# xissburg/edyn

Hardware: AMD Instinct MI355X
Metric: steps/sec (whole node), 32k-box pile, 10 SI iters; HBM GB/s in solve (higher is better)
Workload: dtype f32

## Files before the change

edyn_amd/_capi.py:

```python
import ctypes as C
import os
import numpy as np

_HERE = os.path.dirname(os.path.abspath(__file__))
LIB_PATH = os.environ.get("EDYNHIP_LIB") or os.path.join(_HERE, "libedynhip.so")


class EdynHipError(RuntimeError):
    def __init__(self, code, msg):
        super().__init__(f"edynhip error {code}: {msg}")
        self.code = code


class Config(C.Structure):
    _fields_ = [("device", C.c_int32), ("max_bodies", C.c_uint32), ("max_manifolds", C.c_uint32),
                ("max_joints", C.c_uint32), ("fixed_dt", C.c_float), ("num_velocity_iterations", C.c_uint32),
                ("num_position_iterations", C.c_uint32), ("gravity", C.c_float * 3), ("flags", C.c_uint32)]


class Bodies(C.Structure):
    _fields_ = [("kind", C.c_void_p), ("pos", C.c_void_p), ("orn", C.c_void_p), ("linvel", C.c_void_p),
                ("angvel", C.c_void_p), ("mass", C.c_void_p), ("inertia", C.c_void_p), ("has_inertia", C.c_void_p),
                ("shape_type", C.c_void_p), ("shape_param", C.c_void_p), ("friction", C.c_void_p),
                ("restitution", C.c_void_p), ("group", C.c_void_p), ("mask", C.c_void_p), ("gravity", C.c_void_p),
                ("sleeping_disabled", C.c_void_p), ("center_of_mass", C.c_void_p)]


class Joints(C.Structure):
    _fields_ = [("type", C.c_void_p), ("body", C.c_void_p), ("pivot", C.c_void_p), ("axis", C.c_void_p), ("params", C.c_void_p)]


class Params(C.Structure):
    _fields_ = [("fixed_dt", C.c_float), ("num_velocity_iterations", C.c_uint32), ("num_position_iterations", C.c_uint32),
                ("gravity", C.c_float * 3), ("num_restitution_iterations", C.c_uint32),
                ("num_individual_restitution_iterations", C.c_uint32)]


class Timings(C.Structure):
    _fields_ = [(n, C.c_float) for n in ("broadphase_ms", "narrowphase_ms", "islands_ms", "colouring_ms", "prepare_ms",
                                         "solve_velocity_ms", "integrate_ms", "solve_position_ms", "finish_ms", "step_ms")] + \
               [("solve_velocity_launches", C.c_uint32), ("steps", C.c_uint32)]


class Stats(C.Structure):
    _fields_ = [(n, C.c_uint32) for n in ("num_bodies", "num_manifolds", "num_points", "num_active_manifolds",
                                          "num_islands", "num_colours", "num_joint_colours", "colour_rounds",
                                          "num_joints", "num_joint_rows", "solve_schedule")] + [("colour_size", C.c_uint32 * 64)]


class WorldStats(C.Structure):
    _fields_ = [(n, C.c_uint32) for n in ("num_shards", "num_bodies", "steps", "approach_checks", "repartitions")] + [("bodies_per_shard", C.c_uint32 * 16), ("rebalances", C.c_uint32)]


class WorldEditStats(C.Structure):
    _fields_ = [(n, C.c_uint32) for n in ("edits", "in_place", "shard_rebuilds", "repartitions_by_edit", "approach_checks_by_edit")]


SCHEDULE_NAMES = {0: "none", 1: "k_contact_solve_df2 (dataflow, one launch per step, two lanes per manifold)",
                  2: "k_contact_solve_df (dataflow, one launch per step, one lane per manifold)",
                  3: "k_island_velocity (island-fused: one wave per island)",
                  4: "k_contact_solve_df2 + k_island_velocity (mixed: dataflow launch for islands without joints, one wave per jointed island)",
                  5: "k_contact_solve<WARM,PUSH> / k_joint_solve (one launch per colour and sweep)",
                  6: "k_contact_solve_df4 (dataflow, one launch per step, four lanes per manifold)"}


POINT_DTYPE = np.dtype([
    ("pivotA", np.float32, 3), ("pivotB", np.float32, 3), ("normal", np.float32, 3),
    ("local_normal", np.float32, 3), ("distance", np.float32), ("friction", np.float32),
    ("restitution", np.float32), ("attachment", np.int32), ("lifetime", np.uint32),
    ("normal_impulse", np.float32), ("friction_impulse", np.float32, 2)])
MANIFOLD_DTYPE = np.dtype([
    ("body", np.uint32, 2), ("num_points", np.uint32), ("colour", np.uint32), ("pt", POINT_DTYPE, 4)])

FLAG_TIMING, FLAG_SLEEPING, FLAG_EXCLUSIVE_DEVICE, FLAG_TIMING_SOLVE, FLAG_CONTACT_EVENTS = 1, 4, 8, 16, 32
FLAG_FUSED_VELOCITY_ROWS, FLAG_BLOCK_POSITION = 64, 128
PAIR_FILTER = C.CFUNCTYPE(C.c_int, C.c_void_p, C.c_uint32, C.c_uint32)
EVENT_DTYPE = np.dtype([("type", np.uint32), ("step", np.uint32), ("body", np.uint32, 2), ("point_id", np.uint64)])
EVENT_MANIFOLD_CREATED, EVENT_MANIFOLD_DESTROYED, EVENT_POINT_CREATED, EVENT_POINT_DESTROYED = 1, 2, 3, 4
RECORD_DTYPE = np.dtype([("pos", np.float32, 3), ("orn", np.float32, 4), ("linvel", np.float32, 3), ("angvel", np.float32, 3),
                         ("present_pos", np.float32, 3), ("present_orn", np.float32, 4), ("origin", np.float32, 3), ("flags", np.uint32)])
RECORD_DYNAMIC, RECORD_ASLEEP, RECORD_HAS_ORIGIN, RECORD_REMOVED = 1, 2, 4, 8
RAYCAST_HIT_DTYPE = np.dtype([("body", np.uint32), ("fraction", np.float32), ("normal", np.float32, 3), ("feature", np.int32),
                              ("feature_index", np.uint32), ("reserved", np.uint32)])
RAYCAST_NONE, RAYCAST_BOX_FACE, RAYCAST_CYLINDER_FACE, RAYCAST_CYLINDER_SIDE_EDGE = 0, 1, 2, 3
RAYCAST_CAPSULE_HEMISPHERE, RAYCAST_CAPSULE_SIDE, RAYCAST_POLYHEDRON_FACE = 4, 5, 6
RAYCAST_BRUTE_FORCE = 1
QUERY_PROCEDURAL, QUERY_NON_PROCEDURAL, QUERY_ISLANDS = 0, 1, 2
QUERY_CATEGORIES = {"procedural": QUERY_PROCEDURAL, "non_procedural": QUERY_NON_PROCEDURAL, "islands": QUERY_ISLANDS}
QUERY_BRUTE_FORCE = 1


class RecordView(C.Structure):
    _fields_ = [("records", C.c_void_p), ("num_bodies", C.c_uint32), ("step_index", C.c_uint32), ("events", C.c_void_p),
                ("num_events", C.c_uint32), ("total_events", C.c_uint32)]
STAGE_BROADPHASE, STAGE_NARROWPHASE, STAGE_ISLANDS, STAGE_SOLVE, STAGE_ALL = 1, 2, 4, 8, 15
PATH_BITS = {"COMPACT_DIRECT": 1 << 0, "COMPACT_LIBRARY": 1 << 1, "SORT_DIRECT": 1 << 2, "SORT_LIBRARY": 1 << 3, "SPECULATE": 1 << 4,
             "INPLACE": 1 << 5, "LISTS_FORCED": 1 << 6, "LOOKAHEAD_CHANGED": 1 << 7, "RELABEL_COMPRESS0": 1 << 8,
             "RELABEL_COMPRESS1": 1 << 9, "RELABEL_COMPRESSN": 1 << 10, "VEL_XCD": 1 << 11, "POS_XCD": 1 << 12, "VEL_LANES1": 1 << 13,
             "VEL_LANES2": 1 << 14, "VEL_LANES4": 1 << 15, "VEL_MULTI_ROUND": 1 << 16, "POS_MULTI_ROUND": 1 << 17,
             "POS_COLOUR_PUSH": 1 << 18, "MIXED": 1 << 19, "ISLAND_FUSED": 1 << 20, "PER_COLOUR": 1 << 21, "POLY_ONE_LANE": 1 << 22,
             "POLY_AXES8": 1 << 23, "POLY_AXES16": 1 << 24, "POLY_CONTACTS4": 1 << 25, "POLY_CONTACTS8": 1 << 26,
             "POLY_CONTACTS16": 1 << 27, "POLY_HINTS": 1 << 28, "RECORDS_DIRECT": 1 << 29, "RECORDS_COPY": 1 << 30,
             "WORLD_SERIAL": 1 << 31, "VEL_NAP": 1 << 32}

SYMBOLS = ["edynhip_create", "edynhip_destroy", "edynhip_last_error", "edynhip_set_stream", "edynhip_set_bodies",
           "edynhip_set_joints", "edynhip_step", "edynhip_run_stages", "edynhip_synchronize", "edynhip_get_state",
           "edynhip_set_state", "edynhip_pack_state_device", "edynhip_get_derived", "edynhip_num_manifolds",
           "edynhip_get_manifolds", "edynhip_set_manifolds", "edynhip_get_pairs", "edynhip_get_joint_impulses",
           "edynhip_get_timings", "edynhip_get_stats", "edynhip_abi_version", "edynhip_set_pair_filter", "edynhip_default_should_collide", "edynhip_debug_collide", "edynhip_add_bodies", "edynhip_get_asleep", "edynhip_wake_all", "edynhip_wake_bodies", "edynhip_set_center_of_mass",
           "edynhip_refresh_derived", "edynhip_exclude_collision", "edynhip_remove_collision_exclusion", "edynhip_add_joints",
           "edynhip_remove_joints", "edynhip_set_joint_params", "edynhip_remove_bodies", "edynhip_get_params", "edynhip_set_params",
           "edynhip_step_timed", "edynhip_get_contact_events", "edynhip_get_point_ids", "edynhip_snapshot", "edynhip_snapshot_read", "edynhip_snapshot_records", "edynhip_snapshot_map", "edynhip_set_event_prefetch", "edynhip_prefetched_events",
           "edynhip_set_material_extras", "edynhip_get_point_extras", "edynhip_set_joint_definition",
           "edynhip_set_generic_definition", "edynhip_get_joint_slot_impulses", "edynhip_set_material_ids", "edynhip_insert_material_mixing",
           "edynhip_measure_bandwidth", "edynhip_set_joint_warm_start", "edynhip_set_asleep", "edynhip_create_convex_mesh",
           "edynhip_get_convex_mesh",
           "edynhip_world_create", "edynhip_world_destroy", "edynhip_world_last_error", "edynhip_world_create_convex_mesh",
           "edynhip_world_set_bodies", "edynhip_world_set_joints", "edynhip_world_set_joint_definition", "edynhip_world_exclude_collision",
           "edynhip_world_step", "edynhip_world_get_state", "edynhip_world_get_partition", "edynhip_world_repartition",
           "edynhip_world_get_manifolds", "edynhip_world_get_stats", "edynhip_world_context", "edynhip_partition_islands",
           "edynhip_island_boxes_overlap", "edynhip_get_island_boxes",
           "edynhip_world_set_pair_filter", "edynhip_world_default_should_collide", "edynhip_get_sleep_timers", "edynhip_set_sleep_timers",
           "edynhip_raycast", "edynhip_raycast_device",
           "edynhip_query_aabb", "edynhip_query_aabb_device", "edynhip_query_aabb_stats",
           "edynhip_world_raycast", "edynhip_world_raycast_device", "edynhip_world_query_aabb", "edynhip_world_query_aabb_device",
           "edynhip_world_get_contact_events", "edynhip_world_get_point_ids",
           "edynhip_debug_paths", "edynhip_world_debug_paths",
           "edynhip_world_add_bodies", "edynhip_world_remove_bodies", "edynhip_world_add_joints", "edynhip_world_remove_joints",
           "edynhip_world_edit_joint", "edynhip_world_edit_exclusion", "edynhip_world_set_state", "edynhip_world_get_params",
           "edynhip_world_set_params", "edynhip_world_get_edit_stats", "edynhip_world_get_asleep"]

_lib = None


def lib():
    global _lib
    if _lib is None:
        if not os.path.exists(LIB_PATH):
            raise ImportError(f"{LIB_PATH} is missing - build it with __graft_entry__.build() (make -C edyn_amd/csrc); "
                              "there is no fallback path")
        L = C.CDLL(LIB_PATH)
        L.edynhip_create.restype = C.c_void_p
        L.edynhip_create.argtypes = [C.POINTER(Config), C.POINTER(C.c_int)]
        L.edynhip_destroy.argtypes = [C.c_void_p]
        L.edynhip_last_error.restype = C.c_char_p
        L.edynhip_last_error.argtypes = [C.c_void_p]
        L.edynhip_set_stream.argtypes = [C.c_void_p, C.c_void_p]
        L.edynhip_set_bodies.argtypes = [C.c_void_p, C.c_uint32, C.POINTER(Bodies)]
        L.edynhip_set_joints.argtypes = [C.c_void_p, C.c_uint32, C.POINTER(Joints)]
        L.edynhip_step.argtypes = [C.c_void_p, C.c_uint32]
        L.edynhip_run_stages.argtypes = [C.c_void_p, C.c_uint32]
        L.edynhip_synchronize.argtypes = [C.c_void_p]
        L.edynhip_get_state.argtypes = [C.c_void_p] + [C.c_void_p] * 4
        L.edynhip_set_state.argtypes = [C.c_void_p] + [C.c_void_p] * 4
        L.edynhip_pack_state_device.argtypes = [C.c_void_p, C.c_void_p, C.c_uint32, C.c_uint32]
        L.edynhip_get_derived.argtypes = [C.c_void_p] + [C.c_void_p] * 3
        L.edynhip_raycast.argtypes = [C.c_void_p, C.c_uint32, C.c_void_p, C.c_void_p, C.c_uint32, C.c_void_p, C.c_uint32, C.c_void_p]
        L.edynhip_raycast_device.argtypes = [C.c_void_p, C.c_uint32, C.c_void_p, C.c_void_p, C.c_uint32, C.c_void_p, C.c_uint32, C.c_void_p]
# ... 99 lines not shown
```

edyn_amd/csrc/capi.hip:

```cpp
#include "ctx.hpp"
#include "dpolyhedron.hpp"
#include <algorithm>
#include <atomic>
#include <chrono>
#include <cstdio>
#include <cstring>

namespace eh {
using namespace dm;

static std::string g_create_error;

int set_error(edynhip_ctx *c, int code, const char *what, hipError_t e) {
    std::string msg = what ? what : "";
    if (e != hipSuccess) { msg += ": "; msg += hipGetErrorString(e); }
    if (c) c->err = msg; else g_create_error = msg;
    return code;
}

namespace {
enum KnobKind { KNOB_ON, KNOB_OFF, KNOB_SET, KNOB_NUM, KNOB_PATH };
struct KnobRow {
    const char *name; KnobKind kind; long def;
    bool Knobs::*flag; long Knobs::*num; std::string Knobs::*path;
// ... 43 lines not shown
        case KNOB_SET: k.*r.flag = e != nullptr; break;
        case KNOB_NUM: k.*r.num = e ? atol(e) : r.def; break;
        case KNOB_PATH: k.*r.path = e ? e : ""; break;
        }
    }
    return k;
}

__global__ void k_publish_counters(const uint32_t *__restrict__ src, uint32_t *dst, uint32_t words, volatile uint32_t *seq, uint32_t value) {
    for (uint32_t i = threadIdx.x; i < words; i += blockDim.x) dst[i] = src[i];
    __threadfence_system();
    __syncthreads();
    if (threadIdx.x == 0) { __hip_atomic_store((uint32_t *)seq, value, __ATOMIC_RELEASE, __HIP_MEMORY_SCOPE_SYSTEM); }
}
int publish_counters(edynhip_ctx *c, size_t bytes, uint32_t *ticket) {
    const uint32_t value = ++c->cnt_seq_next;
    c->last_fetch_step = c->step_index;
    hipLaunchKernelGGL(k_publish_counters, dim3(1), dim3(256), 0, c->stream, (const uint32_t *)c->cnt, (uint32_t *)c->cnt_host,
                       (uint32_t)(bytes / sizeof(uint32_t)), c->cnt_seq, value);
    EH_HIP(c, hipGetLastError());
    *ticket = value;
    return EDYNHIP_OK;
}
int wait_counters(edynhip_ctx *c, uint32_t value) {
    const auto t0 = std::chrono::steady_clock::now();
    for (uint32_t spins = 0; *c->cnt_seq != value; ++spins) {
        __builtin_ia32_pause();
        if ((spins & 0xFFFFu) == 0xFFFFu && std::chrono::steady_clock::now() - t0 > std::chrono::seconds(2)) {
            EH_HIP(c, hipStreamSynchronize(c->stream));
            if (*c->cnt_seq != value) return set_error(c, EDYNHIP_ERR_INTERNAL, "fetch_counters: the published sequence number never arrived");
            break;
        }
    }
    std::atomic_thread_fence(std::memory_order_acquire);
    return EDYNHIP_OK;
}
int fetch_counters(edynhip_ctx *c, size_t bytes) {
    uint32_t ticket = 0;
    EH_TRY(publish_counters(c, bytes, &ticket));
    return wait_counters(c, ticket);
}

template <typename T>
static int dalloc(edynhip_ctx *c, T *&p, size_t count) {
    void *q = nullptr;
    size_t bytes = std::max<size_t>(count, 1) * sizeof(T);
    EH_HIP(c, hipMalloc(&q, bytes));
    EH_HIP(c, hipMemsetAsync(q, 0, bytes, c->stream));
    c->allocs.push_back(q);
    p = (T *)q;
    return EDYNHIP_OK;
}

static int alloc_manifolds(edynhip_ctx *c, Manifolds &m, uint32_t cap, uint32_t nb) {
    m.cap = cap;
    if (c->cfg.flags & EDYNHIP_FLAG_CONTACT_EVENTS) EH_TRY(dalloc(c, m.pid, (size_t)cap * kMaxPts));
    EH_TRY(dalloc(c, m.seg_start, nb)); EH_TRY(dalloc(c, m.seg_end, nb)); EH_TRY(dalloc(c, m.prev_idx, cap)); EH_TRY(dalloc(c, m.tree, cap));
    EH_TRY(dalloc(c, m.skey, cap)); EH_TRY(dalloc(c, m.bodyA, cap)); EH_TRY(dalloc(c, m.bodyB, cap)); EH_TRY(dalloc(c, m.info, cap));
    if (kPointRecords) {
        float4 *pts = nullptr;
        EH_TRY(dalloc(c, pts, (size_t)cap * kMaxPts * kPointF));
        m.pA = pts; m.pB = pts + 1; m.nrm = pts + 2; m.lnrm = pts + 3; m.imp = pts + 4;
    } else {
        EH_TRY(dalloc(c, m.pA, (size_t)cap * kMaxPts)); EH_TRY(dalloc(c, m.pB, (size_t)cap * kMaxPts));
        EH_TRY(dalloc(c, m.nrm, (size_t)cap * kMaxPts)); EH_TRY(dalloc(c, m.lnrm, (size_t)cap * kMaxPts));
        EH_TRY(dalloc(c, m.imp, (size_t)cap * kMaxPts));
    }
    return EDYNHIP_OK;
}

static int allocate(edynhip_ctx *c) {
    const uint32_t nb = c->cfg.max_bodies, M = c->cfg.max_manifolds, nj = c->cfg.max_joints;
    Bodies &b = c->b;
    b.cap = nb;
    EH_TRY(dalloc(c, b.xf, (size_t)nb * 8)); EH_TRY(dalloc(c, b.dvw, (size_t)nb * 2)); EH_TRY(dalloc(c, b.linvel, nb)); EH_TRY(dalloc(c, b.angvel, nb));
    EH_TRY(dalloc(c, b.amin, nb)); EH_TRY(dalloc(c, b.amax, nb)); EH_TRY(dalloc(c, b.shape, nb)); EH_TRY(dalloc(c, b.grav, nb));
    EH_TRY(dalloc(c, b.mat, nb)); EH_TRY(dalloc(c, b.mat2, nb)); EH_TRY(dalloc(c, b.flags, nb)); EH_TRY(dalloc(c, b.group, nb)); EH_TRY(dalloc(c, b.mask, nb));
    EH_TRY(dalloc(c, b.island, nb));
    EH_TRY(alloc_manifolds(c, c->m[0], M, nb));
    EH_TRY(alloc_manifolds(c, c->m[1], M, nb));
    Rows &r = c->rows;
    EH_TRY(dalloc(c, r.order, M)); EH_TRY(dalloc(c, r.bA, M)); EH_TRY(dalloc(c, r.bB, M)); EH_TRY(dalloc(c, r.np, M)); EH_TRY(dalloc(c, r.label, M));
    EH_TRY(dalloc(c, r.rw, (size_t)M * kMaxPts * kRowsPerPoint * kRowF));
    EH_TRY(dalloc(c, r.dslot, ((size_t)M + 64) * 4));
    EH_TRY(dalloc(c, r.pslot, ((size_t)M + 32) * 6));
    EH_TRY(dalloc(c, r.next, (size_t)M * 2)); EH_TRY(dalloc(c, r.im, (size_t)M * 2));
    EH_TRY(dalloc(c, r.pw, (size_t)M * kMaxPts * kPosF));
    EH_TRY(dalloc(c, r.slot_of, (size_t)nb * kMaxColours)); EH_TRY(dalloc(c, r.first_slot, nb)); EH_TRY(dalloc(c, r.skip, M));
    LBVH &t = c->bvh;
    EH_TRY(dalloc(c, t.keys, nb)); EH_TRY(dalloc(c, t.keys_sorted, nb));
    EH_TRY(dalloc(c, t.parent, (size_t)2 * nb)); EH_TRY(dalloc(c, t.left, nb)); EH_TRY(dalloc(c, t.right, nb));
    EH_TRY(dalloc(c, t.nmin, (size_t)2 * nb)); EH_TRY(dalloc(c, t.nmax, (size_t)2 * nb)); EH_TRY(dalloc(c, t.visit, nb));
    EH_TRY(dalloc(c, t.np_list, nb)); EH_TRY(dalloc(c, t.rope, (size_t)2 * nb)); EH_TRY(dalloc(c, t.split, 8));
    EH_TRY(dalloc(c, t.cand_list, (size_t)nb * kListCap)); EH_TRY(dalloc(c, t.cand_count, nb)); EH_TRY(dalloc(c, t.ref_min, nb)); EH_TRY(dalloc(c, t.ref_max, nb));
    EH_TRY(dalloc(c, c->np_ra, (size_t)M * kMaxPts)); EH_TRY(dalloc(c, c->np_rb, (size_t)M * kMaxPts)); EH_TRY(dalloc(c, c->np_rn, (size_t)M * kMaxPts));
    EH_TRY(dalloc(c, c->np_rnum, M));
    if (c->cfg.flags & EDYNHIP_FLAG_CONTACT_EVENTS) {
        c->event_cap = 5u * M + 1024u;
        EH_TRY(dalloc(c, c->events, c->event_cap)); EH_TRY(dalloc(c, c->event_count, 4)); EH_TRY(dalloc(c, c->prev_matched, M));
    }
    EH_TRY(dalloc(c, c->pair_keys, M)); EH_TRY(dalloc(c, c->pair_keys_sorted, M)); EH_TRY(dalloc(c, c->new_edges, M)); EH_TRY(dalloc(c, c->new_edge_m, M));
    EH_TRY(dalloc(c, c->isl_top, nb)); EH_TRY(dalloc(c, c->rot_off, nb)); EH_HIP(c, hipMemsetAsync(c->rot_off, 0xFF, (size_t)nb * sizeof(uint32_t), c->stream));
    EH_TRY(dalloc(c, c->own_keys, (size_t)nb * kOwnCap)); EH_TRY(dalloc(c, c->own_count, (size_t)nb + 1)); EH_TRY(dalloc(c, c->own_offset, (size_t)nb + 1));
    EH_TRY(dalloc(c, c->col_keys, M)); EH_TRY(dalloc(c, c->col_keys_sorted, M));
    EH_TRY(dalloc(c, c->col_unc, kColUncCap));
    { const size_t cs = 256 * (((size_t)M + 1023) / 1024) + 1; EH_TRY(dalloc(c, c->cs_hist, cs)); EH_TRY(dalloc(c, c->cs_start, cs)); EH_TRY(dalloc(c, c->cs_sup, 16 * 256)); EH_HIP(c, hipMemset(c->cs_sup, 0, 16 * 256 * sizeof(uint32_t))); }
    EH_TRY(dalloc(c, c->used, nb)); EH_TRY(dalloc(c, c->best[0], nb)); EH_TRY(dalloc(c, c->best[1], nb));
    EH_TRY(dalloc(c, c->com_store, nb)); EH_TRY(dalloc(c, c->origin_store, nb));
    EH_TRY(dalloc(c, c->isl_cnt, (size_t)nb + 1)); EH_TRY(dalloc(c, c->isl_off, (size_t)nb + 1)); EH_TRY(dalloc(c, c->isl_list, nb));
    EH_TRY(dalloc(c, c->isl_items, (size_t)M + nj)); EH_TRY(dalloc(c, c->isl_sorted, (size_t)M + nj)); EH_TRY(dalloc(c, c->isl_joint, nb));
    EH_TRY(dalloc(c, c->isl_err, nb)); EH_TRY(dalloc(c, c->isl_done, nb)); EH_TRY(dalloc(c, c->pos_err, (size_t)nb * kMaxDfPosIters));
    EH_TRY(dalloc(c, c->state_dev, (size_t)nb * 13));
    EH_HIP(c, hipHostMalloc((void **)&c->state_host, (size_t)nb * 13 * sizeof(float), hipHostMallocDefault));
    EH_TRY(dalloc(c, c->sleep_state, nb)); EH_TRY(dalloc(c, c->sleep_action, nb)); EH_TRY(dalloc(c, c->sleep_since, nb));
    EH_TRY(dalloc(c, c->sleep_old_label, nb)); EH_TRY(dalloc(c, c->sleep_size, nb)); EH_TRY(dalloc(c, c->sleep_best, nb)); EH_TRY(dalloc(c, c->sleep_carried, nb));
    EH_HIP(c, hipMemsetAsync(c->sleep_since, 0xFF, (size_t)nb * sizeof(double), c->stream));
    Joints &j = c->j;
    j.cap = nj;
    EH_TRY(dalloc(c, j.orig, nj)); EH_TRY(dalloc(c, j.type, nj)); EH_TRY(dalloc(c, j.bodyA, nj)); EH_TRY(dalloc(c, j.bodyB, nj));
    EH_TRY(dalloc(c, j.pivA, nj)); EH_TRY(dalloc(c, j.pivB, nj)); EH_TRY(dalloc(c, j.axA, nj)); EH_TRY(dalloc(c, j.pA, nj));
    EH_TRY(dalloc(c, j.qA, nj)); EH_TRY(dalloc(c, j.axB, nj)); EH_TRY(dalloc(c, j.pB, nj)); EH_TRY(dalloc(c, j.impulse, (size_t)nj * kJointSlots));
    EH_TRY(dalloc(c, j.wbx, nj)); EH_TRY(dalloc(c, j.gJ, (size_t)nj * 18)); EH_TRY(dalloc(c, j.params, (size_t)nj * kJointParams)); EH_TRY(dalloc(c, j.angle, nj)); EH_TRY(dalloc(c, j.rmask, nj));
    EH_TRY(dalloc(c, j.rA, nj)); EH_TRY(dalloc(c, j.rB, nj)); EH_TRY(dalloc(c, j.wp, nj)); EH_TRY(dalloc(c, j.wq, nj)); EH_TRY(dalloc(c, j.wax, nj));
    EH_TRY(dalloc(c, j.eff, (size_t)nj * kJointSlots)); EH_TRY(dalloc(c, j.rhs, (size_t)nj * kJointSlots));
    EH_TRY(dalloc(c, j.lo, (size_t)nj * kJointSlots)); EH_TRY(dalloc(c, j.hi, (size_t)nj * kJointSlots));
    c->sort_tmp_bytes = sort_temp_bytes(std::max(std::max(M, nb + 1), 256u * ((M + 1023u) / 1024u) + 1u));
    { void *q = nullptr; EH_HIP(c, hipMalloc(&q, c->sort_tmp_bytes)); c->allocs.push_back(q); c->sort_tmp = q; }
    EH_TRY(dalloc(c, c->cnt, 1));
    EH_HIP(c, hipHostMalloc((void **)&c->cnt_host, sizeof(Counters), hipHostMallocDefault));
    std::memset(c->cnt_host, 0, sizeof(Counters));
    { void *q = nullptr; EH_HIP(c, hipHostMalloc(&q, 64, hipHostMallocDefault)); std::memset(q, 0, 64); c->cnt_seq = (volatile uint32_t *)q; }
    EH_HIP(c, hipStreamSynchronize(c->stream));
    return EDYNHIP_OK;
}

struct RawBodies {
    const int32_t *kind; const float *pos, *orn, *linvel, *angvel, *mass, *inertia; const uint8_t *has_inertia;
    const int32_t *shape_type; const float *shape_param, *friction, *restitution; const uint64_t *group, *mask; const float *gravity; const uint8_t *sleeping_disabled; const float *com;
};
__global__ void k_init_bodies(uint32_t first, uint32_t n, RawBodies r, Bodies b, float3 default_gravity, dc::Meshes meshes) {
    const uint32_t l = blockIdx.x * blockDim.x + threadIdx.x;
    if (l >= n) return;
    const uint32_t i = first + l;
    const int kind = r.kind[l], st = r.shape_type[l];
    const f3 pos = mk3(r.pos[3 * l], r.pos[3 * l + 1], r.pos[3 * l + 2]);
    const q4 orn{r.orn[4 * l], r.orn[4 * l + 1], r.orn[4 * l + 2], r.orn[4 * l + 3]};
    const float4 sp = make_float4(r.shape_param[4 * l], r.shape_param[4 * l + 1], r.shape_param[4 * l + 2], r.shape_param[4 * l + 3]);
    float inv_m = 0;
    m3 il = m3_zero(), iw = m3_zero();
    const f3 com = r.com ? mk3(r.com[3 * l], r.com[3 * l + 1], r.com[3 * l + 2]) : mk3(0, 0, 0);
    const bool has_com = !(com.x == 0 && com.y == 0 && com.z == 0);
    if (kind == EDYNHIP_KIND_DYNAMIC) {
        const float mass = r.mass[l];
        inv_m = 1.0f / mass;
        m3 I;
        if (r.has_inertia && r.has_inertia[l]) {
            const float *p = r.inertia + 9 * l;
            I = {{p[0], p[1], p[2]}, {p[3], p[4], p[5]}, {p[6], p[7], p[8]}};
        } else if (st == dc::SHAPE_BOX) {
            f3 ext = from4(sp) * 2.0f;
            f3 d = 1.0f / 12.0f * mass * mk3(ext.y * ext.y + ext.z * ext.z, ext.z * ext.z + ext.x * ext.x, ext.x * ext.x + ext.y * ext.y);
            I = {{d.x, 0, 0}, {0, d.y, 0}, {0, 0, d.z}};
        } else if (st == dc::SHAPE_SPHERE) {
            float s = 0.4f * mass * sp.x * sp.x;
            I = {{1 * s, 0 * s, 0 * s}, {0 * s, 1 * s, 0 * s}, {0 * s, 0 * s, 1 * s}};
        } else if (st == dc::SHAPE_CAPSULE) {
// ... 1689 lines not shown
```

edyn_amd/csrc/ctx.hpp:

```cpp
#pragma once
#include <hip/hip_runtime.h>
#include <cstdint>
#include <functional>
#include <string>
#include <array>
#include <map>
#include <vector>
#include "../../include/edynhip.h"
#include "dmesh.hpp"

namespace eh {

constexpr uint32_t kNoColour = 0xFFu;
constexpr uint32_t kMaxColours = 64;
constexpr uint32_t kMaxContactColours = 63;
constexpr uint32_t kSerialColour = 62;
constexpr int kMaxPts = 4;

constexpr uint32_t BF_KIND_MASK = 0x3u;
constexpr uint32_t BF_SHAPE_SHIFT = 4;
constexpr uint32_t BF_SHAPE_MASK = 0xF0u;
constexpr uint32_t BF_ASLEEP = 0x100u;
constexpr uint32_t BF_NOSLEEP = 0x200u;
constexpr uint32_t BF_REMOVED = 0x400u;
// ... 29 lines not shown
    uint32_t *seg_start = nullptr, *seg_end = nullptr;
    uint32_t *prev_idx = nullptr;
    uint8_t *tree = nullptr;
    float4 *pA = nullptr;
    float4 *pB = nullptr;
    float4 *nrm = nullptr;
    float4 *lnrm = nullptr;
    float4 *imp = nullptr;
    uint64_t *pid = nullptr;
    float4 *xmat = nullptr;
    float4 *ximp = nullptr;
};
constexpr bool kPointRecords = true;
constexpr int kPointF = 5;
__host__ __device__ __forceinline__ size_t pt_at(uint32_t cap, uint32_t k, uint32_t m) {
    return kPointRecords ? ((size_t)m * 4 + k) * kPointF : (size_t)k * cap + m;
}
__host__ __device__ __forceinline__ size_t slot_at(uint32_t cap, uint32_t k, uint32_t m) { return (size_t)k * cap + m; }
constexpr int kXRowF = 3, kXRows = 3, kXPoint = kXRows * kXRowF + 1;

__device__ __forceinline__ const float *mix_lookup(const Bodies &b, uint32_t body0, uint32_t body1) {
    if (b.mix_K == 0) return nullptr;
    const uint32_t c0 = b.mat_cid[body0], c1 = b.mat_cid[body1];
    if (c0 == 0xFFFFFFFFu || c1 == 0xFFFFFFFFu) return nullptr;
    const int32_t e = b.mix_lut[(size_t)c0 * b.mix_K + c1];
    return e < 0 ? nullptr : b.mix_vals + 6 * (size_t)e;
}

struct ContactEvent { uint32_t type, step, bodyA, bodyB; uint64_t pid; };
struct EventSink { ContactEvent *buf; uint32_t *count; uint32_t cap; uint32_t step; uint32_t tag; };
__device__ __forceinline__ void emit_event(const EventSink &ev, uint32_t type, uint32_t a, uint32_t b, uint64_t pid) {
    const uint32_t i = atomicAdd(ev.count, 1u);
    if (i < ev.cap) ev.buf[i] = ContactEvent{type, ev.step, a, b, pid};
}

constexpr int kJointSlots = 24, kJointParams = 64, kJointApiParams = 10, kJointApiSlots = 9, kJointBaseSlots = 9;
struct Joints {
    uint32_t n = 0, cap = 0, num_colours = 0, rows = 0;
    uint32_t *orig = nullptr;
    uint32_t *type = nullptr, *bodyA = nullptr, *bodyB = nullptr;
    float4 *pivA = nullptr, *pivB = nullptr;
    float4 *axA = nullptr;
    float4 *pA = nullptr, *qA = nullptr;
    float4 *axB = nullptr, *pB = nullptr;
    float *params = nullptr;
    float *angle = nullptr;
    float *impulse = nullptr;
    float4 *rA = nullptr, *rB = nullptr;
    float4 *wp = nullptr, *wq = nullptr;
    float4 *wax = nullptr;
    float4 *wbx = nullptr;
    float4 *gJ = nullptr;
    float *eff = nullptr, *rhs = nullptr;
    float *lo = nullptr, *hi = nullptr;
    uint32_t *rmask = nullptr;
    uint32_t colour_start[kMaxColours + 1] = {0};
};
struct HostJoint {
    int32_t type = 0;
    uint32_t body[2] = {0, 0};
    float pivot[6] = {0}, axis[6] = {0};
    float frame[18] = {0};
    bool has_frames = false;
    float params[kJointParams] = {0};
    float impulse[kJointSlots] = {0};
    float angle = 0;
    bool alive = true;
};

struct Rows {
    uint32_t *order = nullptr;
    uint32_t *bA = nullptr, *bB = nullptr, *np = nullptr;
    uint32_t *label = nullptr;
    float4 *rw = nullptr;
    float4 *rwx = nullptr;
    float4 *dslot = nullptr;
    uint32_t *next = nullptr;
    float4 *pslot = nullptr;
    float *im = nullptr;
    float4 *pw = nullptr;
    uint32_t *slot_of = nullptr;
    uint32_t *first_slot = nullptr;
    uint8_t *skip = nullptr;
};
constexpr int kRowF = 5, kRowsPerPoint = 3, kPosF = 4;
constexpr uint32_t kColUncCap = 16384;
constexpr uint32_t kHeadBit = 0x80000000u, kSlotMask = 0x7FFFFFFFu;
__host__ __device__ inline size_t dslot_at(uint32_t slot, uint32_t half) {
    const uint32_t p = slot >> 1, side = slot & 1u;
    return ((size_t)(p >> 6) << 8) + (((side << 1) + half) << 6) + (p & 63u);
}
__host__ __device__ inline size_t pslot_at(uint32_t slot, uint32_t piece) {
    const uint32_t p = slot >> 1;
    return (size_t)(p >> 5) * 192u + (piece << 6) + (slot & 63u);
}

struct Knobs {
    bool dataflow, dataflow_pos, island_fused, mixed, df_xcd;
    long df_lanes, df_waves, dfp_waves, df_nap;
    std::string df_trace, dfp_trace;
    long df_trace_step;
    bool speculate, inplace, bp_lists, bp_adapt, direct_compact, direct_sort, col_lds, np_fused;
    long cc_compress;
    bool poly_hint;
    long poly_group, poly_group2;
    long query_scan_ratio, records_direct;
    bool world_serial, world_trace;
    bool bp_stats, pp_prof, tree_stats;
};

struct RayTree;
struct QueryAabb;

struct LBVH {
    uint64_t *keys = nullptr, *keys_sorted = nullptr;
    uint32_t *parent = nullptr;
    uint32_t *left = nullptr, *right = nullptr;
    uint32_t *rope = nullptr;
    uint32_t *split = nullptr;
    uint32_t *cand_list = nullptr, *cand_count = nullptr;
    float4 *ref_min = nullptr, *ref_max = nullptr;
    bool lists_dirty = true;
    float lookahead = 6.0f;
    uint32_t rebuild_hist = 0;
    float4 *nmin = nullptr, *nmax = nullptr;
    uint32_t *visit = nullptr;
    uint32_t *np_list = nullptr;
    uint32_t num_proc = 0, num_np = 0;
    uint32_t age = 0;
};

struct CandLists { uint32_t *list; uint32_t *count; float4 *ref_min, *ref_max; };
constexpr uint32_t kListCap = 128;
constexpr int kOwnCap = 64;
constexpr uint32_t kListOverflow = 0xFFFFFFFFu;

constexpr uint32_t kMaxDfPosIters = 8;

struct Counters {
    uint32_t num_pairs;
    uint32_t pair_overflow;
    uint32_t num_points;
    uint32_t num_active;
    uint32_t uncoloured;
    uint32_t colour_overflow;
    uint32_t num_islands;
    uint32_t pairs_changed;
    uint32_t num_found;
    uint32_t num_new;
    uint32_t num_extra;
    uint32_t num_awake;
    uint32_t unc_count;
    uint32_t bp_rebuild;
    uint32_t df_abort;
    uint32_t pairs_differ;
    uint32_t isl_num;
    uint32_t isl_max_items;
    uint32_t isl_max_jitems;
    uint32_t isl_free;
    uint32_t tree_found;
    uint32_t tree_marks;
    uint32_t tree_total;
    uint32_t col_wg_rounds;
    uint32_t bp_rebuilt;
    int32_t bounds_min[3], bounds_max[3];
    uint32_t colour_start[4 * kMaxColours], colour_end[4 * kMaxColours];
// ... 213 lines not shown
```

edyn_amd/csrc/solver.hip:

```cpp
#include <mutex>
#include "dstep.hpp"
#include "dpolyhedron.hpp"

namespace eh {

struct BRef { f3 pos, org; q4 orn; f3 v, w; float inv_m; m3 inv_I; };
DI BRef load_bref(const Bodies &b, uint32_t i) {
    BRef r;
    float4 p = B_POS(b, i);
    uint32_t fl = b.flags[i];
    r.pos = from4(p); r.org = B_ORG(b, i); r.orn = q_from4(B_ORN(b, i));
    if (is_dynamic(fl)) {
        r.inv_m = p.w;
        r.inv_I = {from4(B_IW(b, i, 0)), from4(B_IW(b, i, 1)), from4(B_IW(b, i, 2))};
    } else { r.inv_m = 0; r.inv_I = m3_zero(); }
    if ((fl & BF_KIND_MASK) == EDYNHIP_KIND_STATIC) { r.v = mk3(0, 0, 0); r.w = mk3(0, 0, 0); }
    else { r.v = from4(b.linvel[i]); r.w = from4(b.angvel[i]); }
    return r;
}
DI float eff_mass(f3 J0, f3 J1, f3 J2, f3 J3, float imA, const m3 &iA, float imB, const m3 &iB) {
    float s = dot(J0, J0) * imA + dot(mul(iA, J1), J1) + dot(J2, J2) * imB + dot(mul(iB, J3), J3);
    return 1.0f / s;
}
DI float rel_speed(f3 J0, f3 J1, f3 J2, f3 J3, f3 vA, f3 wA, f3 vB, f3 wB) {
    return dot(J0, vA) + dot(J1, wA) + dot(J2, vB) + dot(J3, wB);
}

__global__ void k_solve_begin(uint32_t n, Bodies b, float dt, uint32_t *first_slot) {
    uint32_t i = blockIdx.x * blockDim.x + threadIdx.x;
    if (i < n) solve_begin_body(i, b, dt, first_slot);
}

DI void store_row(float4 *rw, size_t base, size_t cap, f3 Jl, f3 JaA, f3 JaB, float eff, float rhs, float imp, float mu,
                  const BRef &A, const BRef &B) {
    rw[base] = to4(Jl, eff);
    rw[base + cap] = to4(JaA, rhs);
    rw[base + 2 * cap] = to4(JaB, imp);
    rw[base + 3 * cap] = to4(mul(A.inv_I, JaA), mu);
    rw[base + 4 * cap] = to4(mul(B.inv_I, JaB), kLarge);
}
template <bool EXTRAS>
__global__ void k_prep_contacts(uint32_t n_active, Rows rows, uint32_t rcap, Manifolds mf, Bodies b, float dt,
                                const uint32_t *__restrict__ keys_sorted, bool push, bool by_key, bool write_pw) {
    uint32_t p = blockIdx.x * blockDim.x + threadIdx.x;
    if (p >= n_active) return;
    if (by_key && keys_sorted[p] >= 4u * kMaxContactColours) return;
    const uint32_t m = rows.order[p];
    const uint32_t np = mf.info[m] & 0xFF;
    const uint32_t ia = mf.bodyA[m], ib = mf.bodyB[m];
    rows.bA[p] = ia; rows.bB[p] = ib; rows.np[p] = np;
    rows.label[p] = b.island[is_dynamic(b.flags[ia]) ? ia : ib];
    if (push) {
        const uint32_t col = keys_sorted[p] >> 2;
        if (is_dynamic(b.flags[ia])) rows.slot_of[(size_t)ia * kMaxColours + col] = 2 * p;
        if (is_dynamic(b.flags[ib])) rows.slot_of[(size_t)ib * kMaxColours + col] = 2 * p + 1;
    }
    const BRef A = load_bref(b, ia), B = load_bref(b, ib);
    for (uint32_t k = 0; k < np; ++k) {
        const size_t s = slot_at(mf.cap, k, m), t = pt_at(mf.cap, k, m);
        const float4 a4 = mf.pA[t], b4 = mf.pB[t], n4 = mf.nrm[t], im = mf.imp[t];
        const f3 n = from4(n4);
        const float distance = a4.w, mu = b4.w;
        const f3 pAw = to_world(from4(a4), A.org, A.orn), pBw = to_world(from4(b4), B.org, B.orn);
        const f3 rA = pAw - A.pos, rB = pBw - B.pos;
        const f3 J0 = n, J1 = cross(rA, n), J2 = -n, J3 = -cross(rB, n);
        const float effn = eff_mass(J0, J1, J2, J3, A.inv_m, A.inv_I, B.inv_m, B.inv_I);
        const float relvel = rel_speed(J0, J1, J2, J3, A.v, A.w, B.v, B.w);
        float error = distance > 0 ? distance / dt : 0.0f;
        float upper = kLarge;
        float4 xm = make_float4(0, 0, kLarge, kLarge), xi = make_float4(0, 0, 0, 0);
        if (EXTRAS) { xm = mf.xmat[s]; xi = mf.ximp[s]; }
        if (EXTRAS && distance < 0 && xm.z < kLarge) {
            const f3 vA = A.v + cross(A.w, rA), vB = B.v + cross(B.w, rB);
            const float normal_relvel = dot(vA - vB, n);
            const float spring_force = -distance * xm.z / (float)np;
            const float damper_force = -normal_relvel * xm.w / (float)np;
            upper = fmaxf(spring_force + damper_force, 0.0f) * dt;
            error = -kLarge;
        }
        const float rhsn = -(error * 0.2f + relvel * (1 + 0.0f));
        f3 t0, t1;
        plane_space(n, t0, t1);
        const f3 K1 = cross(rA, t0), K3 = -cross(rB, t0);
        const f3 L1 = cross(rA, t1), L3 = -cross(rB, t1);
        const float eff0 = eff_mass(t0, K1, -t0, K3, A.inv_m, A.inv_I, B.inv_m, B.inv_I);
        const float eff1 = eff_mass(t1, L1, -t1, L3, A.inv_m, A.inv_I, B.inv_m, B.inv_I);
        const float rhs0 = -rel_speed(t0, K1, -t0, K3, A.v, A.w, B.v, B.w);
        const float rhs1 = -rel_speed(t1, L1, -t1, L3, A.v, A.w, B.v, B.w);
        const size_t base = (size_t)(k * kRowsPerPoint) * kRowF * rcap + p, rstride = (size_t)kRowF * rcap;
        store_row(rows.rw, base, rcap, n, J1, J3, effn, rhsn, im.x, mu, A, B);
        if (!EXTRAS && push && write_pw) {
            const size_t pb = (size_t)(k * kPosF) * rcap + p;
            rows.pw[pb] = a4; rows.pw[pb + rcap] = b4; rows.pw[pb + 2 * (size_t)rcap] = mf.lnrm[t]; rows.pw[pb + 3 * (size_t)rcap] = n4;
        }
        if (EXTRAS && upper != kLarge) rows.rw[base + 4 * (size_t)rcap].w = upper;
        if (EXTRAS) {
            const size_t xb = (size_t)(k * kXPoint) * rcap + p;
            rows.rwx[xb + 9 * (size_t)rcap] = make_float4(xm.x, xm.y, 0, 0);
            auto axial = [&](int r, f3 ax, float imp, bool guarded) {
                const f3 ia = mul(A.inv_I, ax), ib = mul(B.inv_I, -ax);
                const float ssum = dot(ia, ax) + dot(ib, -ax);
                const float eff = guarded ? (ssum > kEps ? 1.0f / ssum : 0.0f) : 1.0f / ssum;
                const float rhs = guarded ? -rel_speed(mk3(0, 0, 0), ax, mk3(0, 0, 0), -ax, A.v, A.w, B.v, B.w) : -(dot(ax, A.w) + dot(-ax, B.w));
                rows.rwx[xb + (size_t)(3 * r) * rcap] = to4(ax, eff);
                rows.rwx[xb + (size_t)(3 * r + 1) * rcap] = to4(ia, rhs);
                rows.rwx[xb + (size_t)(3 * r + 2) * rcap] = to4(ib, imp);
            };
            if (xm.x > 0) {
                f3 ax0 = t0, ax1 = t1;
                const uint32_t fa = b.flags[ia], fb = b.flags[ib];
#pragma unroll
                for (int side = 0; side < 2; ++side) {
                    const uint32_t fl = side ? fb : fa;
                    if (is_dynamic(fl) && (((fl & BF_SHAPE_MASK) >> BF_SHAPE_SHIFT) == (uint32_t)dc::SHAPE_CAPSULE || ((fl & BF_SHAPE_MASK) >> BF_SHAPE_SHIFT) == (uint32_t)dc::SHAPE_CYLINDER)) {
                        const f3 rdw = rotate(A.orn, dc::axis_vector(b.shape[side ? ib : ia].z));
                        ax0 *= dot(rdw, ax0); ax1 *= dot(rdw, ax1);
                    }
                }
                axial(0, ax0, xi.x, true); axial(1, ax1, xi.y, true);
            }
            if (xm.y > 0) axial(2, n, xi.z, false);
        }
        store_row(rows.rw, base + rstride, rcap, t0, K1, K3, eff0, rhs0, im.y, 0.0f, A, B);
        store_row(rows.rw, base + 2 * rstride, rcap, t1, L1, L3, eff1, rhs1, im.z, 0.0f, A, B);
    }
}

struct Delta { f3 dvA, dwA, dvB, dwB; float imA, imB; m3 iA, iB; };
DI void load_delta(const Bodies &b, uint32_t ia, uint32_t ib, Delta &d) {
    float4 va = B_DV(b, ia), vb = B_DV(b, ib);
    d.dvA = from4(va); d.imA = va.w; d.dwA = from4(B_DW(b, ia));
    d.dvB = from4(vb); d.imB = vb.w; d.dwB = from4(B_DW(b, ib));
    d.iA = {from4(B_IW(b, ia, 0)), from4(B_IW(b, ia, 1)), from4(B_IW(b, ia, 2))};
    d.iB = {from4(B_IW(b, ib, 0)), from4(B_IW(b, ib, 1)), from4(B_IW(b, ib, 2))};
}
DI void store_delta(const Bodies &b, uint32_t ia, uint32_t ib, const Delta &d) {
    if (d.imA != 0) { B_DV(b, ia) = to4(d.dvA, d.imA); B_DW(b, ia) = to4(d.dwA, 0); }
    if (d.imB != 0) { B_DV(b, ib) = to4(d.dvB, d.imB); B_DW(b, ib) = to4(d.dwB, 0); }
}
DI void apply_impulse(Delta &d, f3 J0, f3 J1, f3 J2, f3 J3, float imp) {
    d.dvA += d.imA * J0 * imp;
    d.dvB += d.imB * J2 * imp;
    d.dwA += mul(d.iA, J1) * imp;
    d.dwB += mul(d.iB, J3) * imp;
}

struct RowReg { float4 f[kRowF]; };
DI float dot3_fma(f3 a, f3 b) { return __builtin_fmaf(a.z, b.z, __builtin_fmaf(a.y, b.y, a.x * b.x)); }
DI f3 fma3(f3 w, float s, f3 acc) { return mk3(__builtin_fmaf(w.x, s, acc.x), __builtin_fmaf(w.y, s, acc.y), __builtin_fmaf(w.z, s, acc.z)); }
DI float fused_delta(float rel, float eff, float rhs_eff) { return __builtin_fmaf(-rel, eff, rhs_eff); }
DI float fused_normal(float &cur, float dimp, float upper) {
    const float nw = __builtin_fminf(__builtin_fmaxf(cur + dimp, 0.0f), upper);
    const float applied = nw - cur;
    cur = nw;
    return applied;
}
DI void fused_circle(float &i0, float &i1, float max_len) {
    const float len2 = __builtin_fmaf(i1, i1, i0 * i0);
    if (len2 > max_len * max_len) {
        const float len = sqrtf(len2);
        const float sc = len > kEps ? max_len / len : 0.0f;
        i0 *= sc; i1 *= sc;
    }
}
template <bool FUSED>
DI void row_apply(Delta &d, const RowReg &r, float imp) {
    const f3 Jl = from4(r.f[0]);
    if (FUSED) {
        d.dvA = fma3(d.imA * Jl, imp, d.dvA);
        d.dvB = fma3(d.imB * (-Jl), imp, d.dvB);
        d.dwA = fma3(from4(r.f[3]), imp, d.dwA);
        d.dwB = fma3(from4(r.f[4]), imp, d.dwB);
    } else {
        d.dvA += d.imA * Jl * imp;
        d.dvB += d.imB * (-Jl) * imp;
        d.dwA += from4(r.f[3]) * imp;
        d.dwB += from4(r.f[4]) * imp;
    }
}
template <bool FUSED>
DI float row_relspeed(const Delta &d, const RowReg &r) {
    const f3 Jl = from4(r.f[0]);
    if (FUSED) return (dot3_fma(Jl, d.dvA) + dot3_fma(from4(r.f[1]), d.dwA)) + (dot3_fma(-Jl, d.dvB) + dot3_fma(from4(r.f[2]), d.dwB));
    return rel_speed(Jl, from4(r.f[1]), -Jl, from4(r.f[2]), d.dvA, d.dwA, d.dvB, d.dwB);
}
DI void friction_circle(float &i0, float &i1, float &di0, float &di1, float c0, float c1, float max_len) {
    const float len2 = i0 * i0 + i1 * i1;
    if (len2 > square(max_len)) {
        const float len = sqrtf(len2);
        if (len > kEps) { i0 = i0 / len * max_len; i1 = i1 / len * max_len; }
        else { i0 = 0; i1 = 0; }
        di0 = i0 - c0; di1 = i1 - c1;
    }
}
DI void normal_clamp(float &cur, float &dimp, float upper) {
    const float imp = cur + dimp;
    const bool lt = imp < 0.0f, gt = !lt && imp > upper;
    const float nw = lt ? 0.0f : (gt ? upper : imp);
    dimp = (lt || gt) ? nw - cur : dimp;
    cur = nw;
}
template <class L, bool WARM, bool FUSED>
DI void solve_normal_row(typename L::Acc &x, typename L::Row &r, float upper) {
    if (WARM) { L::template apply<FUSED>(x, r, L::imp(r)); return; }
    if (FUSED) {
        const float applied = fused_normal(L::imp(r), fused_delta(L::template relspeed<true>(x, r), L::eff(r), L::template rhs<true>(r)), upper);
        L::template apply<true>(x, r, applied);
// ... 126 lines not shown
        for (int f = 0; f < kXRowF; ++f) r.f[f] = rwx[xb + (size_t)(6 + f) * rcap];
        if (WARM) { xrow_apply(d, r, r.f[2].w); continue; }
        const float max_len = mu * R[k][0].f[2].w;
        float dimp = (r.f[1].w - xrow_relspeed(d, r)) * r.f[0].w;
        const float cur = r.f[2].w, imp = cur + dimp, lo = -max_len, hi = max_len;
        float out;
        if (imp < lo) { dimp = lo - cur; out = lo; }
        else if (imp > hi) { dimp = hi - cur; out = hi; }
        else out = imp;
        rwx[xb + 8 * (size_t)rcap].w = out;
        xrow_apply(d, r, dimp);
    }
}
template <bool WARM, int NP, bool PUSH, bool FUSED>
DI void contact_solve_np(uint32_t p, uint32_t np, const uint32_t *__restrict__ rbA, const uint32_t *__restrict__ rbB,
                         float4 *__restrict__ rw, uint32_t rcap, float4 *__restrict__ bdvw, const float *__restrict__ im,
                         float4 *__restrict__ rwx = nullptr) {
    uint32_t ia, ib;
    if (PUSH) { ia = rbA[2 * (size_t)p] & kSlotMask; ib = rbA[2 * (size_t)p + 1] & kSlotMask; }
    else { ia = rbA[p]; ib = rbB[p]; }
    RowReg R[NP][kRowsPerPoint];
    rows_load<NP>(R, rw, rcap, p);
    Delta d;
    {
        float4 va, wa, vb, wb;
        if (PUSH) { va = bdvw[dslot_at(2 * p, 0)]; wa = bdvw[dslot_at(2 * p, 1)]; vb = bdvw[dslot_at(2 * p + 1, 0)]; wb = bdvw[dslot_at(2 * p + 1, 1)]; }
        else { va = bdvw[2 * (size_t)ia]; wa = bdvw[2 * (size_t)ia + 1]; vb = bdvw[2 * (size_t)ib]; wb = bdvw[2 * (size_t)ib + 1]; }
        d.dvA = from4(va); d.dwA = from4(wa);
        d.dvB = from4(vb); d.dwB = from4(wb);
        if (PUSH) { d.imA = im[2 * (size_t)p]; d.imB = im[2 * (size_t)p + 1]; }
        else { d.imA = va.w; d.imB = vb.w; }
    }
    rows_solve<WARM, NP, FUSED>(d, R, np);
    if (rwx) extras_solve<WARM, NP>(d, R, np, rwx, rcap, p);
    if (!WARM) rows_store_impulses<NP>(R, rw, rcap, p, np);
    const float wA = PUSH ? 0.0f : d.imA, wB = PUSH ? 0.0f : d.imB;
    const size_t oa0 = PUSH ? dslot_at(ia, 0) : 2 * (size_t)ia, oa1 = PUSH ? dslot_at(ia, 1) : 2 * (size_t)ia + 1;
    const size_t ob0 = PUSH ? dslot_at(ib, 0) : 2 * (size_t)ib, ob1 = PUSH ? dslot_at(ib, 1) : 2 * (size_t)ib + 1;
    if (d.imA != 0) { bdvw[oa0] = to4(d.dvA, wA); bdvw[oa1] = to4(d.dwA, 0); }
    if (d.imB != 0) { bdvw[ob0] = to4(d.dvB, wB); bdvw[ob1] = to4(d.dwB, 0); }
}
template <bool WARM, bool PUSH, bool FUSED>
DI void contact_solve_lane(uint32_t p, uint32_t np, const uint32_t *__restrict__ rbA, const uint32_t *__restrict__ rbB,
                           float4 *__restrict__ rw, uint32_t rcap, float4 *__restrict__ bdvw, const float *__restrict__ im,
                           float4 *__restrict__ rwx = nullptr) {
    if (np > 2) contact_solve_np<WARM, 4, PUSH, FUSED>(p, np, rbA, rbB, rw, rcap, bdvw, im, rwx);
    else contact_solve_np<WARM, 2, PUSH, FUSED>(p, np, rbA, rbB, rw, rcap, bdvw, im, rwx);
}
struct Split { uint32_t e4, e3, e2; };
DI uint32_t np_of(uint32_t p, const Split &sp) { return p < sp.e4 ? 4u : (p < sp.e3 ? 3u : (p < sp.e2 ? 2u : 1u)); }
template <bool WARM, bool PUSH, bool FUSED>
__global__ void __launch_bounds__(64)
k_contact_solve(uint32_t start, uint32_t end, Split sp, const uint32_t *__restrict__ rbA, const uint32_t *__restrict__ rbB,
                float4 *__restrict__ rw, uint32_t rcap, float4 *__restrict__ bdvw, const float *__restrict__ im, float4 *__restrict__ rwx) {
    const uint32_t p = start + blockIdx.x * blockDim.x + threadIdx.x;
    if (p < end) contact_solve_lane<WARM, PUSH, FUSED>(p, np_of(p, sp), rbA, rbB, rw, rcap, bdvw, im, rwx);
}
struct TailRanges { uint32_t n; uint32_t start[kMaxColours]; uint32_t end[kMaxColours]; Split split[kMaxColours]; };
constexpr uint32_t kTailThreads = 256, kTailMax = 512;
template <bool WARM, bool PUSH, bool FUSED>
__global__ void __launch_bounds__(256)
k_contact_solve_tail(TailRanges tr, const uint32_t *rbA, const uint32_t *rbB, float4 *rw, uint32_t rcap, float4 *bdvw, const float *im, float4 *rwx) {
    for (uint32_t c = 0; c < tr.n; ++c) {
        for (uint32_t p = tr.start[c] + threadIdx.x; p < tr.end[c]; p += kTailThreads)
            contact_solve_lane<WARM, PUSH, FUSED>(p, np_of(p, tr.split[c]), rbA, rbB, rw, rcap, bdvw, im, rwx);
        __threadfence_block();
        __syncthreads();
    }
}

typedef float v4f __attribute__((ext_vector_type(4)));
struct DfArgs {
    uint32_t na, stride, sweeps;
    const uint32_t *keys_sorted;
    const uint32_t *next;
    const float *im;
    float4 *rw; uint32_t rcap;
    float4 *dslot;
    Counters *cnt;
    uint64_t *trace;
    const uint8_t *skip;
    uint32_t nap;
    uint32_t xcd_lists;
};
constexpr uint32_t kXcds = 8, kCls = 4 * kMaxColours;
struct XcdLists { uint32_t pre[kCls + 1]; uint32_t first[kCls], lo[kCls], hi[kCls]; };
DI void xcd_lists_build(XcdLists &L, const Counters *cnt, uint32_t g) {
    const uint32_t lane = threadIdx.x & 63u;
    uint32_t n[4], sum = 0;
#pragma unroll
    for (uint32_t k = 0; k < 4; ++k) {
        const uint32_t c = 4 * lane + k, a = cnt->colour_start[c], e = cnt->colour_end[c], size = e > a && c < 4 * kMaxContactColours ? e - a : 0u;
        auto cut = [&](uint32_t i) {
            if (i == 0) return a;
            if (i >= kXcds) return a + size;
            const uint32_t b = (a + (uint32_t)(((uint64_t)size * i) / kXcds) + 16u) & ~31u;
            return b < a ? a : (b > a + size ? a + size : b);
        };
        const uint32_t lo = cut(g), hi = cut(g + 1), v = lo & ~31u;
        L.first[c] = v; L.lo[c] = lo; L.hi[c] = hi;
        n[k] = hi > lo ? ((hi - v) + 31u) & ~31u : 0u;
        sum += n[k];
    }
    uint32_t inc = sum;
#pragma unroll
    for (int d = 1; d < 64; d <<= 1) { const uint32_t u = __shfl_up(inc, d); if ((int)lane >= d) inc += u; }
    uint32_t at = inc - sum;
#pragma unroll
    for (uint32_t k = 0; k < 4; ++k) { L.pre[4 * lane + k] = at; at += n[k]; }
    if (lane == 63) L.pre[kCls] = at;
    __syncthreads();
}
DI uint32_t xcd_lists_p(const XcdLists &L, uint32_t q, uint32_t none) {
    uint32_t lo = 0, hi = kCls;
#pragma unroll 1
    while (hi - lo > 1) { const uint32_t mid = (lo + hi) >> 1; if (L.pre[mid] <= q) lo = mid; else hi = mid; }
    const uint32_t p = L.first[lo] + (q - L.pre[lo]);
    return p >= L.lo[lo] && p < L.hi[lo] ? p : none;
}
DI void df_nap(uint32_t nap) { if (nap == 0) return; if (nap == 1) __builtin_amdgcn_s_sleep(1); else __builtin_amdgcn_s_sleep(4); }
DI void df_poll(const float4 *slot, v4f &a0, v4f &a1, v4f &b0, v4f &b1) {
    asm volatile("global_load_dwordx4 %0, %4, off sc1\n\t"
                 "global_load_dwordx4 %1, %4, off offset:1024 sc1\n\t"
                 "global_load_dwordx4 %2, %4, off offset:2048 sc1\n\t"
                 "global_load_dwordx4 %3, %4, off offset:3072 sc1\n\t"
                 "s_waitcnt vmcnt(0)"
                 : "=&v"(a0), "=&v"(a1), "=&v"(b0), "=&v"(b1) : "v"(slot) : "memory");
}
DI void df_publish(float4 *slot, f3 dv, f3 dw, uint32_t tag) {
    const float t = __uint_as_float(tag);
    const v4f v = {dv.x, dv.y, dv.z, t}, w = {dw.x, dw.y, dw.z, t};
    asm volatile("global_store_dwordx4 %0, %1, off sc1\n\t"
                 "global_store_dwordx4 %0, %2, off offset:1024 sc1" : : "v"(slot), "v"(v), "v"(w) : "memory");
}
constexpr uint32_t kDfSpinLimit = 1u << 22;
template <bool WARM, int NP, bool FUSED>
DI void df_task(const DfArgs &a, uint32_t p, bool valid, uint32_t np, uint32_t col, uint32_t sweep, uint64_t *trace_slot) {
    constexpr int kEarly = NP > 2 ? 2 : NP;
    RowReg Rn[NP], Rf[NP][2];
    const uint64_t w0 = a.trace ? wall_clock64() : 0;
#pragma unroll
    for (int k = 0; k < NP; ++k) row_load(Rn[k], a.rw, a.rcap, p, k, 0);
#pragma unroll
    for (int k = 0; k < kEarly; ++k) { row_load(Rf[k][0], a.rw, a.rcap, p, k, 1); row_load(Rf[k][1], a.rw, a.rcap, p, k, 2); }
    uint64_t w1 = 0, w2 = 0;
    const uint32_t nA = a.next[2 * (size_t)p], nB = a.next[2 * (size_t)p + 1];
    Delta d;
    d.imA = a.im[2 * (size_t)p]; d.imB = a.im[2 * (size_t)p + 1];
    d.dvA = d.dwA = d.dvB = d.dwB = mk3(0, 0, 0);
    const uint32_t wantA = (nA & kHeadBit) ? sweep : sweep + 1, wantB = (nB & kHeadBit) ? sweep : sweep + 1;
    bool gotA = d.imA == 0, gotB = d.imB == 0;
    bool done = !valid;
    const float4 *mine = a.dslot + dslot_at(2 * p, 0);
    for (uint32_t spin = 0;; ++spin) {
        if (!done && !(gotA && gotB)) {
            v4f a0, a1, b0, b1;
            df_poll(mine, a0, a1, b0, b1);
            if (a.trace && w1 == 0) w1 = wall_clock64();
            if (!gotA && __float_as_uint(a0.w) == wantA && __float_as_uint(a1.w) == wantA) {
                d.dvA = mk3(a0.x, a0.y, a0.z); d.dwA = mk3(a1.x, a1.y, a1.z); gotA = true;
            }
            if (!gotB && __float_as_uint(b0.w) == wantB && __float_as_uint(b1.w) == wantB) {
                d.dvB = mk3(b0.x, b0.y, b0.z); d.dwB = mk3(b1.x, b1.y, b1.z); gotB = true;
            }
        }
        const uint64_t pending = __ballot(!done);
        if (pending == 0) {
            if (trace_slot && (threadIdx.x & 63) == 0) { trace_slot[0] = w0; trace_slot[1] = w1; trace_slot[2] = w2; trace_slot[3] = wall_clock64(); }
            break;
        }
        const uint32_t minc = __shfl(col, __ffsll((long long)pending) - 1);
        const bool mine_now = !done && col == minc;
        if (__ballot(mine_now && !(gotA && gotB)) == 0) {
            if (a.trace && w2 == 0) w2 = wall_clock64();
            if (mine_now) {
#pragma unroll
                for (int k = kEarly; k < NP; ++k) { row_load(Rf[k][0], a.rw, a.rcap, p, k, 1); row_load(Rf[k][1], a.rw, a.rcap, p, k, 2); }
                rows_solve_normals<WARM, NP, FUSED>(d, Rn, np);
#pragma unroll
                for (int k = 0; k < NP; ++k)
                    if ((uint32_t)k < np) solve_friction_pair<Lanes1, WARM, FUSED>(d, Rf[k][0], Rf[k][1], Rn[k].f[3].w, Rn[k].f[2].w);
                if (d.imA != 0) df_publish(a.dslot + dslot_at(nA & kSlotMask, 0), d.dvA, d.dwA, sweep + 1);
                if (d.imB != 0) df_publish(a.dslot + dslot_at(nB & kSlotMask, 0), d.dvB, d.dwB, sweep + 1);
                if (!WARM) {
#pragma unroll
                    for (int k = 0; k < NP; ++k) {
                        if ((uint32_t)k >= np) continue;
                        a.rw[(size_t)((k * kRowsPerPoint + 0) * kRowF + 2) * a.rcap + p] = Rn[k].f[2];
                        a.rw[(size_t)((k * kRowsPerPoint + 1) * kRowF + 2) * a.rcap + p] = Rf[k][0].f[2];
                        a.rw[(size_t)((k * kRowsPerPoint + 2) * kRowF + 2) * a.rcap + p] = Rf[k][1].f[2];
                    }
                }
                done = true;
            }
        } else {
            if (spin > kDfSpinLimit || ((spin & 1023u) == 1023u && __hip_atomic_load(&a.cnt->df_abort, __ATOMIC_RELAXED, __HIP_MEMORY_SCOPE_AGENT))) {
                if (spin > kDfSpinLimit) atomicExch(&a.cnt->df_abort, 1u);
                break;
            }
            __builtin_amdgcn_s_sleep(4);
        }
    }
}
constexpr uint32_t kDfBlock = 64;
template <bool FUSED>
__global__ void __launch_bounds__(kDfBlock) k_contact_solve_df(DfArgs a) {
    const uint32_t t = blockIdx.x * 64u + threadIdx.x;
    const uint32_t rounds = (a.na + a.stride - 1) / a.stride, nwaves = a.stride >> 6;
    for (uint32_t sweep = 0; sweep < a.sweeps; ++sweep)
        for (uint32_t base = 0, round = 0; base < a.na; base += a.stride, ++round) {
            const uint32_t pt = base + t;
            const bool valid = pt < a.na && !(a.skip && a.skip[pt]);
            if (!__any(valid)) continue;
            const uint32_t p = valid ? pt : a.na - 1;
            const uint32_t key = a.keys_sorted[p];
            const uint32_t np = 4u - (key & 3u), col = key >> 2;
            const bool big = __any(valid && np > 2);
            uint64_t *tr = a.trace ? a.trace + 4 * ((size_t)(sweep * rounds + round) * nwaves + blockIdx.x) : nullptr;
            if (sweep == 0) { if (big) df_task<true, 4, FUSED>(a, p, valid, np, col, sweep, tr); else df_task<true, 2, FUSED>(a, p, valid, np, col, sweep, tr); }
            else { if (big) df_task<false, 4, FUSED>(a, p, valid, np, col, sweep, tr); else df_task<false, 2, FUSED>(a, p, valid, np, col, sweep, tr); }
        }
}

__global__ void k_push_links(uint32_t n_active, Rows rows, const uint32_t *__restrict__ keys_sorted, Bodies b, const uint64_t *__restrict__ used,
                             const uint32_t *__restrict__ isl_joint) {
    uint32_t p = blockIdx.x * blockDim.x + threadIdx.x;
    if (p >= n_active) return;
    if (isl_joint) {
        const bool fused = isl_joint[rows.label[p]] != 0;
        rows.skip[p] = fused ? 1 : 0;
        if (fused) return;
    }
    const uint32_t col = keys_sorted[p] >> 2;
#pragma unroll
    for (uint32_t side = 0; side < 2; ++side) {
        const uint32_t body = side ? rows.bB[p] : rows.bA[p];
        const uint32_t slot = 2 * p + side;
        rows.dslot[dslot_at(slot, 0)] = make_float4(0, 0, 0, 0); rows.dslot[dslot_at(slot, 1)] = make_float4(0, 0, 0, 0);
        if (!is_dynamic(b.flags[body])) {
            rows.next[slot] = slot;
            rows.im[slot] = 0.0f;
            continue;
        }
        rows.im[slot] = B_POS(b, body).w;
        const uint64_t mask = used[body];
        const uint64_t above = col >= 63 ? 0ull : mask & ~((2ull << col) - 1ull);
        const uint32_t nextc = (uint32_t)__ffsll((long long)(above ? above : mask)) - 1;
        const bool head = col == (uint32_t)__ffsll((long long)mask) - 1;
        rows.next[slot] = rows.slot_of[(size_t)body * kMaxColours + nextc] | (head ? kHeadBit : 0u);
        if (head) rows.first_slot[body] = slot;
    }
}

DI void store_impulses_of(uint32_t p, const Rows &rows, uint32_t rcap, const Manifolds &mf) {
    const uint32_t m = rows.order[p], np = rows.np[p];
    for (uint32_t k = 0; k < np; ++k) {
        const size_t d = slot_at(mf.cap, k, m), td = pt_at(mf.cap, k, m);
        float4 im = mf.imp[td];
        im.x = rows.rw[(size_t)((k * kRowsPerPoint + 0) * kRowF + 2) * rcap + p].w;
        im.y = rows.rw[(size_t)((k * kRowsPerPoint + 1) * kRowF + 2) * rcap + p].w;
        im.z = rows.rw[(size_t)((k * kRowsPerPoint + 2) * kRowF + 2) * rcap + p].w;
        mf.imp[td] = im;
        if (rows.rwx && mf.ximp) {
            const size_t xb = (size_t)(k * kXPoint) * rcap + p;
            const float4 mu = rows.rwx[xb + 9 * (size_t)rcap];
            float4 xi = mf.ximp[d];
            if (mu.x > 0) { xi.x = rows.rwx[xb + 2 * (size_t)rcap].w; xi.y = rows.rwx[xb + 5 * (size_t)rcap].w; }
            if (mu.y > 0) xi.z = rows.rwx[xb + 8 * (size_t)rcap].w;
            mf.ximp[d] = xi;
        }
    }
}
__global__ void k_store_impulses(uint32_t n_active, Rows rows, uint32_t rcap, Manifolds mf) {
    uint32_t p = blockIdx.x * blockDim.x + threadIdx.x;
    if (p < n_active) store_impulses_of(p, rows, rcap, mf);
}

DI void joint_rowJ(int type, int r, f3 rA, f3 rB, f3 wp, f3 wq, f3 wax, f3 wbx, f3 &J0, f3 &J1, f3 &J2, f3 &J3) {
    const bool hinge = type == EDYNHIP_JOINT_HINGE;
    if (type == EDYNHIP_JOINT_GRAVITY) {
        J0 = wp; J1 = mk3(0, 0, 0); J2 = -wp; J3 = -mk3(0, 0, 0);
    } else if (type == EDYNHIP_JOINT_DISTANCE || type == EDYNHIP_JOINT_SOFT_DISTANCE || type == EDYNHIP_JOINT_CONE) {
        J0 = wp; J1 = wq; J2 = -wp; J3 = -wax;
    } else if (type == EDYNHIP_JOINT_CVJOINT && r >= 3) {
        J0 = mk3(0, 0, 0); J2 = mk3(0, 0, 0);
        if (r < 7) { J1 = wp; J3 = -wq; }
        else { const f3 ax = r == 7 ? wax : wbx; J1 = ax; J3 = -ax; }
    } else if (r < 3) {
        f3 e = r == 0 ? mk3(1, 0, 0) : (r == 1 ? mk3(0, 1, 0) : mk3(0, 0, 1));
        f3 sa = r == 0 ? mk3(0, -rA.z, rA.y) : (r == 1 ? mk3(rA.z, 0, -rA.x) : mk3(-rA.y, rA.x, 0));
        f3 sb = r == 0 ? mk3(0, -rB.z, rB.y) : (r == 1 ? mk3(rB.z, 0, -rB.x) : mk3(-rB.y, rB.x, 0));
        J0 = e; J1 = -sa; J2 = -e; J3 = sb;
    } else {
        f3 ax = (hinge && r == 3) ? wp : ((hinge && r == 4) ? wq : wax);
        J0 = mk3(0, 0, 0); J1 = ax; J2 = mk3(0, 0, 0); J3 = -ax;
    }
}
DI float atan2_cr(float y, float x) { return (float)atan2((double)y, (double)x); }
DI float normalize_angle(float a) {
    a = fmodf(a, kPi2);
    if (a < -kPi) return a + kPi2;
    if (a > kPi) return a - kPi2;
    return a;
// ... 609 lines not shown
        else if (attach == dc::NA_ON_B) n = sideB ? nrot : nother;
        const float distance = dot(pAw - pBw, n);
        const f3 rX = pXw - X.pos;
        n4[k] = to4(n, n4[k].w);
        piv[k].w = distance;
        if (distance > -kEps) continue;
        if (iw_stale) { const m3 basis = to_m3(X.orn); X.iw = mul(mul(basis, X.il), transpose(basis)); iw_stale = false; }
        const f3 Jl = sideB ? -n : n;
        const f3 cx = cross(rX, n);
        const f3 Ja = sideB ? -cx : cx;
        const f3 iwJa = mul(X.iw, Ja);
        const float t1 = dot(Jl, Jl) * X.inv_m, t2 = dot(iwJa, Ja);
        const float o1 = xchg1(t1), o2 = xchg1(t2);
        const float a1 = sideB ? o1 : t1, a2 = sideB ? o2 : t2, b1 = sideB ? t1 : o1, b2 = sideB ? t2 : o2;
        const float em = 1.0f / (a1 + a2 + b1 + b2);
        const float error = -distance;
        const float corr = error * 0.2f * em;
        max_err = fmaxf(fabsf(error), max_err);
        if (!X.proc) continue;
        X.pos += X.inv_m * Jl * corr;
        X.orn = normalize(X.orn + quaternion_derivative(X.orn, iwJa * corr));
        iw_stale = true;
        if (X.has_com) X.org = to_world(-X.com, X.pos, X.orn); else X.org = X.pos;
        any = true;
    }
    return any;
}
DI void pos_solve(PBody &A, PBody &B, f3 J0, f3 J1, f3 J2, f3 J3, float error, float &max_err) {
    float em = eff_mass(J0, J1, J2, J3, A.inv_m, A.iw, B.inv_m, B.iw);
    float corr = error * 0.2f * em;
    pos_apply(A, J0, J1, corr);
    pos_apply(B, J2, J3, corr);
    pos_origin(A); pos_origin(B);
    max_err = fmaxf(fabsf(error), max_err);
}
DI void publish_error(bool active, float max_err, uint32_t label, float *isl_err) {
    uint32_t rep = active ? label : 0xFFFFFFFFu;
#pragma unroll
    for (int off = 32; off > 0; off >>= 1) rep = min(rep, (uint32_t)__shfl_xor((int)rep, off));
    float m = active ? max_err : 0.0f;
    if (__all(!active || label == rep)) {
#pragma unroll
        for (int off = 32; off > 0; off >>= 1) m = fmaxf(m, __shfl_xor(m, off));
        if ((threadIdx.x & 63) == 0 && m > 0 && rep != 0xFFFFFFFFu) atomicMax((unsigned int *)&isl_err[rep], __float_as_uint(m));
    } else if (m > 0) {
        atomicMax((unsigned int *)&isl_err[label], __float_as_uint(m));
    }
}


struct Row2 { f3 jl, ijl, ja, ija; float eff, rhs, imp; };
DI float dppA(float v) { return __int_as_float(__builtin_amdgcn_update_dpp(0, __float_as_int(v), 0xA0 , 0xF, 0xF, true)); }
DI float dppB(float v) { return __int_as_float(__builtin_amdgcn_update_dpp(0, __float_as_int(v), 0xF5 , 0xF, 0xF, true)); }
DI void df2_poll(const float4 *slot, v4f &h0, v4f &h1) {
    asm volatile("global_load_dwordx4 %0, %2, off sc1\n\t"
                 "global_load_dwordx4 %1, %2, off offset:1024 sc1\n\t"
                 "s_waitcnt vmcnt(0)"
                 : "=&v"(h0), "=&v"(h1) : "v"(slot) : "memory");
}
struct Side { f3 dv, dw; };
template <bool FUSED>
DI float df2_relspeed(const Side &x, const Row2 &r) {
    if (FUSED) {
        const float p = dot3_fma(r.jl, x.dv) + dot3_fma(r.ja, x.dw);
        return p + xchg1(p);
    }
    const float lin = dot(r.jl, x.dv), ang = dot(r.ja, x.dw);
    return dppA(lin) + dppA(ang) + dppB(lin) + dppB(ang);
}
template <bool FUSED>
DI void df2_apply(Side &x, const Row2 &r, float imp) {
    if (FUSED) { x.dv = fma3(r.ijl, imp, x.dv); x.dw = fma3(r.ija, imp, x.dw); }
    else { x.dv += r.ijl * imp; x.dw += r.ija * imp; }
}
struct Lanes2 {
    typedef Side Acc; typedef Row2 Row;
    static constexpr bool kLimitFirst = false;
    template <bool FUSED> static DI float relspeed(const Side &x, const Row2 &r) { return df2_relspeed<FUSED>(x, r); }
    template <bool FUSED> static DI void apply(Side &x, const Row2 &r, float imp) { df2_apply<FUSED>(x, r, imp); }
    static DI float eff(const Row2 &r) { return r.eff; }
    template <bool FUSED> static DI float rhs(const Row2 &r) { return r.rhs; }
    static DI float &imp(Row2 &r) { return r.imp; }
};
template <bool WARM, int NP, bool EXACT, bool FUSED>
DI void df2_task(const DfArgs &a, uint32_t p, bool valid, bool sideB, uint32_t np, uint32_t col, uint32_t sweep, uint64_t *trace_slot) {
    Row2 R[NP][kRowsPerPoint];
    float mu[NP];
    const uint64_t w0 = a.trace ? wall_clock64() : 0;
    const uint32_t slot = 2 * p + (sideB ? 1u : 0u);
    const uint32_t nx = a.next[slot];
    const float im = a.im[slot];
#pragma unroll
    for (int k = 0; k < NP; ++k) {
#pragma unroll
        for (int r = 0; r < kRowsPerPoint; ++r) {
            const size_t base = (size_t)((k * kRowsPerPoint + r) * kRowF) * a.rcap + p;
            const float4 f0 = a.rw[base];
            const float4 fa = a.rw[base + (size_t)(sideB ? 2 : 1) * a.rcap];
            const float4 fi = a.rw[base + (size_t)(sideB ? 4 : 3) * a.rcap];
            Row2 &q = R[k][r];
            const f3 Jl = from4(f0);
            q.jl = sideB ? -Jl : Jl;
            q.ijl = im * q.jl;
            q.ja = from4(fa); q.ija = from4(fi);
            q.eff = f0.w;
            q.rhs = FUSED ? dppA(fa.w) * f0.w : dppA(fa.w); q.imp = dppB(fa.w);
            if (r == 0) mu[k] = dppA(fi.w);
        }
    }
    Side x;
    x.dv = x.dw = mk3(0, 0, 0);
    const uint32_t want = (nx & kHeadBit) ? sweep : sweep + 1;
    bool got = im == 0;
    bool done = !valid;
    const float4 *mine = a.dslot + dslot_at(slot, 0);
    uint64_t w1 = 0, w2 = 0;
    for (uint32_t spin = 0;; ++spin) {
        if (!done && !got) {
            v4f h0, h1;
            df2_poll(mine, h0, h1);
            if (__float_as_uint(h0.w) == want && __float_as_uint(h1.w) == want) {
                x.dv = mk3(h0.x, h0.y, h0.z); x.dw = mk3(h1.x, h1.y, h1.z); got = true;
            }
        }
        if (a.trace && w1 == 0) w1 = wall_clock64();
        const uint64_t pending = __ballot(!done);
        if (pending == 0) {
            if (trace_slot && (threadIdx.x & 63) == 0) { trace_slot[0] = w0; trace_slot[1] = w1; trace_slot[2] = w2; trace_slot[3] = wall_clock64(); }
            break;
        }
        const uint32_t minc = __shfl(col, __ffsll((long long)pending) - 1);
        const bool mine_now = !done && col == minc;
        if (__ballot(mine_now && !got) == 0) {
            if (a.trace && w2 == 0) w2 = wall_clock64();
            if (mine_now) {
#pragma unroll
                for (int k = 0; k < NP; ++k)
                    if (EXACT || (uint32_t)k < np) solve_normal_row<Lanes2, WARM, FUSED>(x, R[k][0], kLarge);
#pragma unroll
                for (int k = 0; k < NP; ++k)
                    if (EXACT || (uint32_t)k < np) solve_friction_pair<Lanes2, WARM, FUSED>(x, R[k][1], R[k][2], mu[k], R[k][0].imp);
                if (im != 0) df_publish(a.dslot + dslot_at(nx & kSlotMask, 0), x.dv, x.dw, sweep + 1);
                if (!WARM && sideB) {
#pragma unroll
                    for (int k = 0; k < NP; ++k) {
                        if (!EXACT && (uint32_t)k >= np) continue;
#pragma unroll
                        for (int r = 0; r < kRowsPerPoint; ++r)
                            a.rw[(size_t)((k * kRowsPerPoint + r) * kRowF + 2) * a.rcap + p] = to4(R[k][r].ja, R[k][r].imp);
                    }
                }
                done = true;
            }
        } else {
            if (spin > kDfSpinLimit || ((spin & 1023u) == 1023u && __hip_atomic_load(&a.cnt->df_abort, __ATOMIC_RELAXED, __HIP_MEMORY_SCOPE_AGENT))) {
                if (spin > kDfSpinLimit) atomicExch(&a.cnt->df_abort, 1u);
                break;
            }
            df_nap(a.nap);
        }
    }
}
template <bool WARM, bool FUSED>
DI void df2_dispatch(const DfArgs &a, uint32_t p, bool valid, bool sideB, uint32_t np, uint32_t col, uint32_t sweep, uint64_t *tr) {
    if (!WARM && __all(!valid || np == 4u)) df2_task<WARM, 4, true, FUSED>(a, p, valid, sideB, np, col, sweep, tr);
    else if (!WARM && __all(!valid || np == 2u)) df2_task<WARM, 2, true, FUSED>(a, p, valid, sideB, np, col, sweep, tr);
    else if (!WARM && __all(!valid || np == 1u)) df2_task<WARM, 1, true, FUSED>(a, p, valid, sideB, np, col, sweep, tr);
    else if (__any(np > 2u)) df2_task<WARM, 4, false, FUSED>(a, p, valid, sideB, np, col, sweep, tr);
    else df2_task<WARM, 2, false, FUSED>(a, p, valid, sideB, np, col, sweep, tr);
}
template <bool FUSED>
__global__ void __launch_bounds__(64) k_contact_solve_df2(DfArgs a) {
    const uint32_t t = blockIdx.x * 32u + (threadIdx.x >> 1);
    const bool sideB = threadIdx.x & 1u;
    if (a.xcd_lists) {
        __shared__ XcdLists L;
        xcd_lists_build(L, a.cnt, blockIdx.x % kXcds);
        const uint32_t count = L.pre[kCls], step = (gridDim.x / kXcds) * 32u, mine = (blockIdx.x / kXcds) * 32u + (threadIdx.x >> 1);
        for (uint32_t sweep = 0; sweep < a.sweeps; ++sweep)
            for (uint32_t base = 0; base < count; base += step) {
                const uint32_t q = base + mine;
                const uint32_t pt = q < count ? xcd_lists_p(L, q, a.na) : a.na;
                const bool valid = pt < a.na && !(a.skip && a.skip[pt]);
                if (!__any(valid)) continue;
                const uint32_t p = pt < a.na ? pt : a.na - 1;
                const uint32_t key = a.keys_sorted[p];
                const uint32_t np = valid ? 4u - (key & 3u) : 0u, col = key >> 2;
                if (sweep == 0) df2_dispatch<true, FUSED>(a, p, valid, sideB, np, col, sweep, nullptr);
                else df2_dispatch<false, FUSED>(a, p, valid, sideB, np, col, sweep, nullptr);
            }
        return;
    }
    const uint32_t rounds = (a.na + a.stride - 1) / a.stride, nwaves = a.stride >> 5;
    for (uint32_t sweep = 0; sweep < a.sweeps; ++sweep)
        for (uint32_t base = 0, round = 0; base < a.na; base += a.stride, ++round) {
            const uint32_t pt = base + t;
            const bool valid = pt < a.na && !(a.skip && a.skip[pt]);
            if (!__any(valid)) continue;
            const uint32_t p = valid ? pt : a.na - 1;
            const uint32_t key = a.keys_sorted[p];
            const uint32_t np = valid ? 4u - (key & 3u) : 0u, col = key >> 2;
            uint64_t *tr = a.trace ? a.trace + 4 * ((size_t)(sweep * rounds + round) * nwaves + blockIdx.x) : nullptr;
            if (sweep == 0) df2_dispatch<true, FUSED>(a, p, valid, sideB, np, col, sweep, tr);
            else df2_dispatch<false, FUSED>(a, p, valid, sideB, np, col, sweep, tr);
        }
}

struct Row4 { f3 j, ij; float eff, rhs, imp; };
DI float qb0(float v) { return __int_as_float(__builtin_amdgcn_update_dpp(0, __float_as_int(v), 0x00 , 0xF, 0xF, true)); }
DI float qb1(float v) { return __int_as_float(__builtin_amdgcn_update_dpp(0, __float_as_int(v), 0x55 , 0xF, 0xF, true)); }
DI float qb2(float v) { return __int_as_float(__builtin_amdgcn_update_dpp(0, __float_as_int(v), 0xAA , 0xF, 0xF, true)); }
DI float qb3(float v) { return __int_as_float(__builtin_amdgcn_update_dpp(0, __float_as_int(v), 0xFF , 0xF, 0xF, true)); }
DI void df4_poll(const float4 *piece, v4f &h) {
    asm volatile("global_load_dwordx4 %0, %1, off sc1\n\t"
                 "s_waitcnt vmcnt(0)"
                 : "=&v"(h) : "v"(piece) : "memory");
}
DI void df4_publish(float4 *piece, f3 d, uint32_t tag) {
    const v4f v = {d.x, d.y, d.z, __uint_as_float(tag)};
    asm volatile("global_store_dwordx4 %0, %1, off sc1" : : "v"(piece), "v"(v) : "memory");
}
DI float xchg2(float v) {
    return __int_as_float(__builtin_amdgcn_update_dpp(0, __float_as_int(v), 0x4E , 0xF, 0xF, true));
}
template <bool FUSED>
DI float df4_relspeed(const f3 &x, const Row4 &r) {
    if (FUSED) {
        const float t = dot3_fma(r.j, x);
        const float side = t + xchg1(t);
        return side + xchg2(side);
    }
    const float t = dot(r.j, x);
    return qb0(t) + qb1(t) + qb2(t) + qb3(t);
}
template <bool FUSED>
DI void df4_apply(f3 &x, const Row4 &r, float imp) { if (FUSED) x = fma3(r.ij, imp, x); else x += r.ij * imp; }
struct Lanes4 {
    typedef f3 Acc; typedef Row4 Row;
    static constexpr bool kLimitFirst = false;
    template <bool FUSED> static DI float relspeed(const f3 &x, const Row4 &r) { return df4_relspeed<FUSED>(x, r); }
    template <bool FUSED> static DI void apply(f3 &x, const Row4 &r, float imp) { df4_apply<FUSED>(x, r, imp); }
    static DI float eff(const Row4 &r) { return r.eff; }
    template <bool FUSED> static DI float rhs(const Row4 &r) { return r.rhs; }
    static DI float &imp(Row4 &r) { return r.imp; }
};
template <bool WARM, int NP, bool EXACT, bool FUSED>
DI void df4_task(const DfArgs &a, uint32_t p, bool valid, uint32_t role, uint32_t np, uint32_t col, uint32_t sweep, uint64_t *trace_slot) {
    Row4 R[NP][kRowsPerPoint];
    float mu[NP];
    const uint64_t w0 = a.trace ? wall_clock64() : 0;
    const uint32_t side = role >> 1;
    const bool ang = role & 1u;
    const uint32_t slot = 2 * p + side;
    const uint32_t nx = a.next[slot];
    const float im = a.im[slot];
    const size_t off_a = (size_t)(ang ? 1u + side : 0u) * a.rcap, off_i = (size_t)(3u + side) * a.rcap;
#pragma unroll
    for (int k = 0; k < NP; ++k) {
#pragma unroll
        for (int r = 0; r < kRowsPerPoint; ++r) {
            const size_t base = (size_t)((k * kRowsPerPoint + r) * kRowF) * a.rcap + p;
            const float4 fa = a.rw[base + off_a];
            float4 fi = fa;
            if (ang) fi = a.rw[base + off_i];
            Row4 &q = R[k][r];
            const f3 Ja = from4(fa);
            q.j = role == 2u ? -Ja : Ja;
            const f3 lin = im * q.j;
            q.ij = ang ? from4(fi) : lin;
            q.eff = qb0(fa.w); q.rhs = FUSED ? qb1(fa.w) * q.eff : qb1(fa.w); q.imp = qb3(fa.w);
            if (r == 0) mu[k] = qb1(fi.w);
        }
    }
    f3 x = mk3(0, 0, 0);
    const uint32_t want = (nx & kHeadBit) ? sweep : sweep + 1;
    bool got = im == 0;
    bool done = !valid;
    const float4 *mine = a.dslot + dslot_at(slot, ang ? 1u : 0u);
    uint64_t w1 = 0, w2 = 0;
    for (uint32_t spin = 0;; ++spin) {
        if (!done && !got) {
            v4f h;
            df4_poll(mine, h);
            if (__float_as_uint(h.w) == want) { x = mk3(h.x, h.y, h.z); got = true; }
        }
        if (a.trace && w1 == 0) w1 = wall_clock64();
        const uint64_t pending = __ballot(!done);
        if (pending == 0) {
            if (trace_slot && (threadIdx.x & 63) == 0) { trace_slot[0] = w0; trace_slot[1] = w1; trace_slot[2] = w2; trace_slot[3] = wall_clock64(); }
            break;
        }
        const uint32_t minc = __shfl(col, __ffsll((long long)pending) - 1);
        const bool mine_now = !done && col == minc;
        if (__ballot(mine_now && !got) == 0) {
            if (a.trace && w2 == 0) w2 = wall_clock64();
            if (mine_now) {
#pragma unroll
                for (int k = 0; k < NP; ++k)
                    if (EXACT || (uint32_t)k < np) solve_normal_row<Lanes4, WARM, FUSED>(x, R[k][0], kLarge);
#pragma unroll
                for (int k = 0; k < NP; ++k)
                    if (EXACT || (uint32_t)k < np) solve_friction_pair<Lanes4, WARM, FUSED>(x, R[k][1], R[k][2], mu[k], R[k][0].imp);
                if (im != 0) df4_publish(a.dslot + dslot_at(nx & kSlotMask, ang ? 1u : 0u), x, sweep + 1);
                if (!WARM && role == 3u) {
#pragma unroll
                    for (int k = 0; k < NP; ++k) {
                        if (!EXACT && (uint32_t)k >= np) continue;
#pragma unroll
                        for (int r = 0; r < kRowsPerPoint; ++r)
                            a.rw[(size_t)((k * kRowsPerPoint + r) * kRowF + 2) * a.rcap + p] = to4(R[k][r].j, R[k][r].imp);
                    }
                }
                done = true;
            }
        } else {
            if (spin > kDfSpinLimit || ((spin & 1023u) == 1023u && __hip_atomic_load(&a.cnt->df_abort, __ATOMIC_RELAXED, __HIP_MEMORY_SCOPE_AGENT))) {
                if (spin > kDfSpinLimit) atomicExch(&a.cnt->df_abort, 1u);
                break;
            }
            __builtin_amdgcn_s_sleep(2);
        }
    }
}
template <bool WARM, bool FUSED>
DI void df4_dispatch(const DfArgs &a, uint32_t p, bool valid, uint32_t role, uint32_t np, uint32_t col, uint32_t sweep, uint64_t *tr) {
    if (!WARM && __all(!valid || np == 4u)) df4_task<WARM, 4, true, FUSED>(a, p, valid, role, np, col, sweep, tr);
    else if (!WARM && __all(!valid || np == 2u)) df4_task<WARM, 2, true, FUSED>(a, p, valid, role, np, col, sweep, tr);
    else if (__any(np > 2u)) df4_task<WARM, 4, false, FUSED>(a, p, valid, role, np, col, sweep, tr);
    else df4_task<WARM, 2, false, FUSED>(a, p, valid, role, np, col, sweep, tr);
}
template <bool FUSED>
__global__ void __launch_bounds__(64) __attribute__((amdgpu_waves_per_eu(2, 2))) k_contact_solve_df4(DfArgs a) {
    const uint32_t t = blockIdx.x * 16u + (threadIdx.x >> 2);
    const uint32_t role = threadIdx.x & 3u;
    const uint32_t rounds = (a.na + a.stride - 1) / a.stride, nwaves = a.stride >> 4;
    for (uint32_t sweep = 0; sweep < a.sweeps; ++sweep)
        for (uint32_t base = 0, round = 0; base < a.na; base += a.stride, ++round) {
            const uint32_t pt = base + t;
            const bool valid = pt < a.na && !(a.skip && a.skip[pt]);
            if (!__any(valid)) continue;
            const uint32_t p = valid ? pt : a.na - 1;
            const uint32_t key = a.keys_sorted[p];
            const uint32_t np = valid ? 4u - (key & 3u) : 0u, col = key >> 2;
            uint64_t *tr = a.trace ? a.trace + 4 * ((size_t)(sweep * rounds + round) * nwaves + blockIdx.x) : nullptr;
            if (sweep == 0) df4_dispatch<true, FUSED>(a, p, valid, role, np, col, sweep, tr);
            else df4_dispatch<false, FUSED>(a, p, valid, role, np, col, sweep, tr);
        }
}
template <int NP, bool BLOCK>
DI void pos_contacts_np(bool in_range, uint32_t pc, bool sideB, uint32_t np, const Rows &rows, const Manifolds &mf, const Bodies &b,
                        float *isl_err, const uint32_t *isl_done, uint32_t m, uint32_t ia, uint32_t ib, uint32_t label) {
    const uint32_t ix = sideB ? ib : ia;
    const float4 *__restrict__ pvsrc = sideB ? mf.pB : mf.pA;
    float4 piv[NP], l4[NP], n4[NP];
#pragma unroll
    for (int k = 0; k < NP; ++k) {
        const size_t s = pt_at(mf.cap, (uint32_t)k, m);
        piv[k] = pvsrc[s]; l4[k] = mf.lnrm[s]; n4[k] = mf.nrm[s];
    }
    PBody X = load_pbody(b, ix);
    const uint32_t done = isl_done[label];
    float max_err = 0;
    bool soft[NP];
#pragma unroll
    for (int k = 0; k < NP; ++k) soft[k] = mf.xmat != nullptr && mf.xmat[(size_t)k * mf.cap + m].z < kLarge;
    bool live[NP];
#pragma unroll
    for (int k = 0; k < NP; ++k) live[k] = (uint32_t)k < np && in_range && !soft[k];
    bool iw_stale = false;
    const bool corrected = BLOCK ? pos_manifold_block<NP>(X, sideB, piv, l4, n4, live, max_err) : pos_manifold_points<NP>(X, sideB, piv, l4, n4, live, max_err, iw_stale);
    if (BLOCK ? corrected : iw_stale) pos_rebuild_inertia(X);
    const bool active = in_range && done == 0;
    if (active) {
#pragma unroll
        for (int k = 0; k < NP; ++k) {
            const size_t s = pt_at(mf.cap, (uint32_t)k, m);
            if ((uint32_t)k < np && !soft[k]) {
                if (!sideB) mf.pA[s] = piv[k];
                else mf.nrm[s] = n4[k];
            }
        }
        store_pbody(b, ix, X);
    }
    publish_error(active && !sideB, max_err, label, isl_err);
}
template <bool BLOCK>
DI void pos_contacts_item(bool in_range, uint32_t pc, bool sideB, const Rows &rows, const Manifolds &mf, const Bodies &b,
                          float *isl_err, const uint32_t *isl_done) {
    const uint32_t m = rows.order[pc];
    const uint32_t ia = rows.bA[pc], ib = rows.bB[pc], np = in_range ? rows.np[pc] : 0;
    const uint32_t label = rows.label[pc];
    if (__any(np > 2)) pos_contacts_np<4, BLOCK>(in_range, pc, sideB, np, rows, mf, b, isl_err, isl_done, m, ia, ib, label);
    else pos_contacts_np<2, BLOCK>(in_range, pc, sideB, np, rows, mf, b, isl_err, isl_done, m, ia, ib, label);
}
template <bool BLOCK>
DI void pos_contacts_lane(uint32_t start, uint32_t end, uint32_t t, const Rows &rows, const Manifolds &mf, const Bodies &b,
                          float *isl_err, const uint32_t *isl_done) {
    const uint32_t p = start + (t >> 1);
    pos_contacts_item<BLOCK>(p < end, p < end ? p : start, t & 1, rows, mf, b, isl_err, isl_done);
}
template <bool BLOCK>
__global__ void __launch_bounds__(128)
k_pos_contacts(uint32_t start, uint32_t end, Rows rows, Manifolds mf, Bodies b, float *isl_err, const uint32_t *__restrict__ isl_done) {
    pos_contacts_lane<BLOCK>(start, end, blockIdx.x * blockDim.x + threadIdx.x, rows, mf, b, isl_err, isl_done);
}
template <bool BLOCK>
__global__ void __launch_bounds__(256)
k_pos_contacts_tail(TailRanges tr, Rows rows, Manifolds mf, Bodies b, float *isl_err, const uint32_t *isl_done) {
    for (uint32_t c = 0; c < tr.n; ++c) {
        for (uint32_t base = tr.start[c]; base < tr.end[c]; base += 128) {
            pos_contacts_lane<BLOCK>(base, tr.end[c], threadIdx.x, rows, mf, b, isl_err, isl_done);
        }
        __threadfence_block();
        __syncthreads();
    }
}
template <bool WARM, bool FUSED>
__global__ void __launch_bounds__(64)
k_contact_solve_serial(uint32_t start, uint32_t end, Split sp, const uint32_t *rbA, const uint32_t *rbB, float4 *rw, uint32_t rcap, float4 *bdvw, float4 *rwx) {
    if (threadIdx.x != 0) return;
    for (uint32_t p = start; p < end; ++p) {
        contact_solve_lane<WARM, false, FUSED>(p, np_of(p, sp), rbA, rbB, rw, rcap, bdvw, nullptr, rwx);
        __threadfence();
    }
}
template <bool BLOCK>
__global__ void __launch_bounds__(64)
k_pos_contacts_serial(uint32_t start, uint32_t end, Rows rows, Manifolds mf, Bodies b, float *isl_err, const uint32_t *isl_done) {
    for (uint32_t p = start; p < end; ++p) {
// ... 557 lines not shown
        b.amax[i] = make_float4(fmaxf(p0.x, p1.x) + sh.x, fmaxf(p0.y, p1.y) + sh.x, fmaxf(p0.z, p1.z) + sh.x, 0);
    } else if (st == dc::SHAPE_CYLINDER) {
        const box3 bb = dc::cylinder_aabb(dc::cyl_of(b.shape[i]), pos, orn);
        b.amin[i] = to4(bb.mn, 0); b.amax[i] = to4(bb.mx, 0);
    } else if (st == dc::SHAPE_POLYHEDRON) {
        const box3 bb = dc::polyhedron_aabb(meshes, b.shape[i], pos, orn);
        b.amin[i] = to4(bb.mn, 0); b.amax[i] = to4(bb.mx, 0);
    }
    if (kind == EDYNHIP_KIND_DYNAMIC) {
        const m3 il = {from4(B_IL(b, i, 0)), from4(B_IL(b, i, 1)), from4(B_IL(b, i, 2))};
        const m3 iw = mul(mul(basis, il), transpose(basis));
        B_IW(b, i, 0) = to4(iw.r0, 0); B_IW(b, i, 1) = to4(iw.r1, 0); B_IW(b, i, 2) = to4(iw.r2, 0);
    }
}
__global__ void k_finish(uint32_t n, Bodies b, uint64_t *used, uint32_t *next_seg_start, uint32_t *next_seg_end, Counters *cnt,
                         const float4 *__restrict__ pslot, const uint32_t *__restrict__ first_slot, CandLists cl, uint32_t *__restrict__ isl_joint, uint2 *__restrict__ isl_top, dc::Meshes meshes) {
    uint32_t i = blockIdx.x * blockDim.x + threadIdx.x;
    if (blockIdx.x == 0) {
        const int t = threadIdx.x;
        if (t == 0) {
            cnt->num_pairs = 0; cnt->pair_overflow = 0; cnt->num_points = 0; cnt->num_active = 0;
            cnt->uncoloured = 0; cnt->colour_overflow = 0; cnt->pairs_changed = 0; cnt->num_found = 0; cnt->num_new = 0; cnt->num_extra = 0; cnt->num_awake = 0; cnt->unc_count = 0; cnt->pairs_differ = 0; cnt->tree_found = 0; cnt->tree_marks = 0;
        }
        if (t < 3) { cnt->bounds_min[t] = 0x7FFFFFFF; cnt->bounds_max[t] = (int)0x80000000; }
        for (int k = t; k < 4 * (int)kMaxColours; k += (int)blockDim.x) { cnt->colour_start[k] = 0; cnt->colour_end[k] = 0; }
    }
    bool moved = false;
    if (i < n) {
        used[i] = 0; next_seg_start[i] = 0; next_seg_end[i] = 0; isl_joint[i] = 0; isl_top[i] = make_uint2(0u, 0u);
        const uint32_t fl = b.flags[i];
        if (pslot && is_dynamic(fl)) pos_writeback(b, i, pslot, first_slot);
        derive_body(b, i, meshes);
        if (cl.count && is_dynamic(fl) && !(fl & BF_REMOVED)) {
            const float4 a = b.amin[i], c = b.amax[i], ra = cl.ref_min[i], rc = cl.ref_max[i];
            const float d = fmaxf(fmaxf(fmaxf(fabsf(a.x - ra.x), fabsf(a.y - ra.y)), fabsf(a.z - ra.z)),
                                  fmaxf(fmaxf(fabsf(c.x - rc.x), fabsf(c.y - rc.y)), fabsf(c.z - rc.z)));
            moved = !(d <= ra.w);
        }
    }
    if (__any(moved) && (threadIdx.x & 63) == 0) cnt->bp_rebuild = 1u;
}
__global__ void k_refresh_derived(uint32_t n, Bodies b, dc::Meshes meshes) {
    uint32_t i = blockIdx.x * blockDim.x + threadIdx.x;
    if (i < n) derive_body(b, i, meshes);
}
int refresh_derived(edynhip_ctx *c) {
    if (c->b.n == 0) return EDYNHIP_OK;
    hipLaunchKernelGGL(k_refresh_derived, dim3((c->b.n + 255) / 256), dim3(256), 0, c->stream, c->b.n, c->b, c->meshes);
    EH_HIP(c, hipGetLastError());
    return EDYNHIP_OK;
}

static hipError_t launch_resident(edynhip_ctx *c, const void *kernel, uint32_t grid, uint32_t block, void **params) {
    if (c->cfg.flags & EDYNHIP_FLAG_EXCLUSIVE_DEVICE) return hipLaunchKernel(kernel, dim3(grid), dim3(block), params, 0, c->stream);
    static std::mutex coop_launch[64], coop_first;
    std::unique_lock<std::mutex> first(coop_first, std::defer_lock);
    if (!c->coop_launched) first.lock();
    std::lock_guard<std::mutex> guard(coop_launch[(uint32_t)c->device & 63u]);
    const hipError_t e = hipLaunchCooperativeKernel(kernel, dim3(grid), dim3(block), params, 0, c->stream);
    c->coop_launched = true;
    return e;
}
static void rec(edynhip_ctx *c, int idx) {
    if (c->timer.e && ((c->timer.mask >> idx) & 1u)) (void)hipEventRecord(c->timer.e[idx], c->stream);
}

using ContactSolveFn = void (*)(uint32_t, uint32_t, Split, const uint32_t *, const uint32_t *, float4 *, uint32_t, float4 *, const float *, float4 *);
using ContactTailFn = void (*)(TailRanges, const uint32_t *, const uint32_t *, float4 *, uint32_t, float4 *, const float *, float4 *);
using ContactSerialFn = void (*)(uint32_t, uint32_t, Split, const uint32_t *, const uint32_t *, float4 *, uint32_t, float4 *, float4 *);
static ContactSolveFn contact_solve_fn(bool warm, bool push, bool fused) {
    static const ContactSolveFn t[2][2][2] = {{{k_contact_solve<false, false, false>, k_contact_solve<false, false, true>}, {k_contact_solve<false, true, false>, k_contact_solve<false, true, true>}},
                                              {{k_contact_solve<true, false, false>, k_contact_solve<true, false, true>}, {k_contact_solve<true, true, false>, k_contact_solve<true, true, true>}}};
    return t[warm][push][fused];
}
static ContactTailFn contact_tail_fn(bool warm, bool push, bool fused) {
    static const ContactTailFn t[2][2][2] = {{{k_contact_solve_tail<false, false, false>, k_contact_solve_tail<false, false, true>}, {k_contact_solve_tail<false, true, false>, k_contact_solve_tail<false, true, true>}},
                                             {{k_contact_solve_tail<true, false, false>, k_contact_solve_tail<true, false, true>}, {k_contact_solve_tail<true, true, false>, k_contact_solve_tail<true, true, true>}}};
    return t[warm][push][fused];
}
static ContactSerialFn contact_serial_fn(bool warm, bool fused) {
    static const ContactSerialFn t[2][2] = {{k_contact_solve_serial<false, false>, k_contact_solve_serial<false, true>}, {k_contact_solve_serial<true, false>, k_contact_solve_serial<true, true>}};
    return t[warm][fused];
}
static const void *df_velocity_fn(uint32_t lanes, bool fused) {
    if (lanes == 4u) return fused ? (const void *)k_contact_solve_df4<true> : (const void *)k_contact_solve_df4<false>;
    if (lanes == 2u) return fused ? (const void *)k_contact_solve_df2<true> : (const void *)k_contact_solve_df2<false>;
    return fused ? (const void *)k_contact_solve_df<true> : (const void *)k_contact_solve_df<false>;
}
static const void *df_position_fn(bool block) { return block ? (const void *)k_pos_contacts_df<true> : (const void *)k_pos_contacts_df<false>; }

static void probe_dataflow(edynhip_ctx *c, bool fused_rows, bool block_pos) {
    c->df_mode = 0;
    int ncu = 0, coop = 0;
    if (c->knobs.dataflow &&
        hipDeviceGetAttribute(&ncu, hipDeviceAttributeMultiprocessorCount, c->device) == hipSuccess &&
        hipDeviceGetAttribute(&coop, hipDeviceAttributeCooperativeLaunch, c->device) == hipSuccess && ncu > 0 && coop) {
        auto resident = [&](const void *fn) {
            int per_cu = 0;
            return hipOccupancyMaxActiveBlocksPerMultiprocessor(&per_cu, fn, kDfBlock, 0) == hipSuccess && per_cu > 0 ? (uint32_t)per_cu * (uint32_t)ncu : 0u;
        };
        for (uint32_t lanes : {1u, 2u, 4u}) c->df_resident[lanes] = resident(df_velocity_fn(lanes, fused_rows));
        c->dfp_waves = resident(df_position_fn(block_pos));
        if (c->df_resident[1] > 0) c->df_mode = 1;
    }
    (void)hipGetLastError();
}

struct SolvePlan {
    bool fused_rows = false, block_pos = false;
    uint32_t na = 0;
    bool serial = false;
    uint32_t nc_par = 0;
    uint32_t first_tail = 0;
    TailRanges tail{};
    bool isl_candidate = false;
    uint32_t largest = 0xFFFFFFFFu;
    bool mixed = false;
    bool isl_fused = false;
    bool push = false;
    uint32_t lanes = 0, vel_grid = 0;
    bool pos_df = false;
    uint32_t pos_grid = 0;
    void set_largest(uint32_t items) { largest = items; isl_fused = isl_candidate && !mixed && largest <= kIslFusedLimit; }
    void drop_dataflow() { lanes = 0; pos_df = false; }
    const uint8_t *df_skip(const edynhip_ctx *c) const { return mixed ? c->rows.skip : nullptr; }
    uint32_t schedule(uint32_t num_joints) const {
        return (na + num_joints) == 0 ? EDYNHIP_SCHEDULE_NONE
               : lanes ? (mixed ? EDYNHIP_SCHEDULE_MIXED : lanes == 4u ? EDYNHIP_SCHEDULE_DATAFLOW4 : lanes == 2u ? EDYNHIP_SCHEDULE_DATAFLOW2 : EDYNHIP_SCHEDULE_DATAFLOW1)
               : isl_fused ? EDYNHIP_SCHEDULE_ISLAND_FUSED : EDYNHIP_SCHEDULE_PER_COLOUR;
    }
};
constexpr bool kPwInPrep = true;
constexpr uint32_t kMixedMinFree = 1024;
constexpr uint32_t kIslGrid = 4096;

static SolvePlan plan_solve(const edynhip_ctx *c) {
    const Knobs &kn = c->knobs;
    const Joints &j = c->j;
    SolvePlan p;
    p.fused_rows = (c->cfg.flags & EDYNHIP_FLAG_FUSED_VELOCITY_ROWS) != 0;
    p.block_pos = (c->cfg.flags & EDYNHIP_FLAG_BLOCK_POSITION) != 0;
    const uint32_t na = p.na = c->num_active, nc = c->num_colours;
    p.serial = nc == kSerialColour + 1 && c->colour_end[kSerialColour] > c->colour_start[kSerialColour];
    p.nc_par = p.serial ? kSerialColour : nc;
    const bool contacts_only = j.n == 0 && !c->extras;
    p.isl_candidate = kn.island_fused && !contacts_only && !p.serial && (na + j.n) > 0 && (size_t)na + j.n < kIslIdMask;
    uint32_t largest = 0xFFFFFFFFu, largest_jointed = 0xFFFFFFFFu, free_manifolds = 0;
    if (p.isl_candidate) {
        const bool fetched = c->last_fetch_step == c->step_index;
        if (fetched && c->isl_prep_step + 1 == c->step_index) {
            largest = c->cnt_host->isl_max_items; largest_jointed = c->cnt_host->isl_max_jitems; free_manifolds = c->cnt_host->isl_free;
        } else if (!fetched && c->isl_cache_epoch == c->topology_epoch) {
            largest = c->isl_cache_max; largest_jointed = c->isl_cache_jmax; free_manifolds = c->isl_cache_free;
        }
    }
    p.mixed = p.isl_candidate && kn.mixed && j.n > 0 && !c->extras && na > 0 && c->df_mode == 1 && c->cfg.num_position_iterations <= kMaxDfPosIters &&
              free_manifolds >= kMixedMinFree && largest_jointed <= kIslFusedLimit && !c->b.com;
    p.set_largest(largest);
    p.push = na > 0 && !p.serial && (contacts_only || p.mixed);
    p.first_tail = p.nc_par;
    while (p.first_tail > 0 && c->colour_end[p.first_tail - 1] - c->colour_start[p.first_tail - 1] <= kTailMax) --p.first_tail;
    if (p.nc_par - p.first_tail >= 2) {
        for (uint32_t k = p.first_tail; k < p.nc_par; ++k)
            if (c->colour_end[k] > c->colour_start[k]) {
                p.tail.start[p.tail.n] = c->colour_start[k]; p.tail.end[p.tail.n] = c->colour_end[k];
                p.tail.split[p.tail.n] = Split{c->colour_split[k][0], c->colour_split[k][1], c->colour_split[k][2]};
                ++p.tail.n;
            }
    } else p.first_tail = p.nc_par;
    if (p.push && c->df_mode == 1) {
        const bool latency_bound = c->df_resident[2] > 0 && na <= 16u * 32u * c->df_resident[2];
        uint32_t lanes = latency_bound ? 2u : 1u;
        if (kn.df_lanes == 1 || kn.df_lanes == 2 || kn.df_lanes == 4) lanes = (uint32_t)kn.df_lanes;
        if (lanes == 4u && c->df_resident[4] == 0) lanes = 2u;
        if (lanes == 2u && c->df_resident[2] == 0) lanes = 1u;
        const uint32_t per_wave = 64u / lanes;
        const uint32_t resident = c->df_resident[lanes];
        const uint32_t want_waves = kn.df_waves ? (uint32_t)kn.df_waves : std::max(lanes == 4u ? 2048u : lanes == 2u ? 1024u : 512u, blocks(na, per_wave * 9));
        p.lanes = lanes;
        p.vel_grid = std::min(blocks(na, per_wave), std::min(resident, want_waves));
    }
    const uint32_t P = c->cfg.num_position_iterations;
    p.pos_df = P > 0 && P <= kMaxDfPosIters && p.push && c->df_mode == 1 && kn.dataflow_pos && !c->b.com;
    if (p.pos_df) p.pos_grid = std::min(blocks(na, 32), std::min(c->dfp_waves, kn.dfp_waves ? (uint32_t)kn.dfp_waves : std::max(p.block_pos ? 512u : 1024u, blocks(na, 32 * 9))));
    return p;
}

static void prep_contacts(edynhip_ctx *c, uint32_t count, bool push, bool by_key, bool pw) {
    const Manifolds &mf = c->m[c->cur];
    if (!c->extras) hipLaunchKernelGGL(k_prep_contacts<false>, dim3(blocks(count, 128)), dim3(128), 0, c->stream, count, c->rows, mf.cap, mf, c->b, c->cfg.fixed_dt, c->col_keys_sorted, push, by_key, pw);
    else hipLaunchKernelGGL(k_prep_contacts<true>, dim3(blocks(count, 128)), dim3(128), 0, c->stream, count, c->rows, mf.cap, mf, c->b, c->cfg.fixed_dt, c->col_keys_sorted, push, by_key, pw);
}

static int bucket_islands(edynhip_ctx *c, SolvePlan &p) {
    hipStream_t s = c->stream;
    const Joints &j = c->j;
    const uint32_t n = c->b.n, na = p.na;
    const IslLists isl{c->isl_cnt, c->isl_off, c->isl_list, c->isl_items, c->isl_sorted, c->isl_joint};
    JointColours jc{};
    jc.n = j.num_colours;
    for (uint32_t k = 0; k <= j.num_colours && k <= kMaxColours; ++k) jc.start[k] = j.colour_start[k];
    const bool keep_lists = na == 0 && !c->sleep_active() && c->isl_lists_epoch == c->topology_epoch;
    if (!keep_lists) {
        EH_HIP(c, hipMemsetAsync(&c->cnt->isl_num, 0, 4 * sizeof(uint32_t), s));
        hipLaunchKernelGGL(k_isl_count, dim3(blocks(j.n + na, 256)), dim3(256), 0, s, j.n, na, j, c->rows, c->b, isl);
        EH_TRY(scan_u32(c, c->isl_cnt, c->isl_off, n + 1));
        hipLaunchKernelGGL(k_isl_fill, dim3(blocks(j.n + na, 256)), dim3(256), 0, s, j.n, na, j, jc, c->rows, c->col_keys_sorted, c->b, isl, c->cnt);
        c->isl_lists_epoch = (na == 0 && !c->sleep_active()) ? c->topology_epoch : 0xFFFFFFFFu;
    }
    if (p.largest == 0xFFFFFFFFu && c->last_fetch_step != c->step_index) {
        EH_TRY(fetch_counters(c, sizeof(Counters) - sizeof(uint32_t) * 8 * kMaxColours));
        p.set_largest(c->isl_cache_max = c->cnt_host->isl_max_items);
        c->isl_cache_jmax = c->cnt_host->isl_max_jitems; c->isl_cache_free = c->cnt_host->isl_free;
        c->isl_cache_epoch = c->topology_epoch;
    }
    c->isl_prep_step = c->step_index;
    if ((p.isl_fused || p.mixed) && !keep_lists) {
        EH_TRY(fetch_counters(c, sizeof(Counters) - sizeof(uint32_t) * 8 * kMaxColours));
        if (p.isl_fused && c->cnt_host->isl_max_items > kIslFusedLimit) p.isl_fused = false;
        if (p.mixed && c->cnt_host->isl_max_jitems > kIslFusedLimit) {
            p.mixed = false; p.push = false; p.drop_dataflow();
            if (na) prep_contacts(c, na, false, false, false);
        }
    }
    return EDYNHIP_OK;
}
static IslSolveArgs island_args(edynhip_ctx *c, const SolvePlan &p, uint32_t iters) {
    const IslLists isl{c->isl_cnt, c->isl_off, c->isl_list, c->isl_items, c->isl_sorted, c->isl_joint};
    return IslSolveArgs{isl, c->cnt, c->j, c->b, c->rows, c->m[c->cur], c->m[c->cur].cap, c->extras ? c->rows.rwx : nullptr, iters, c->isl_err, c->isl_done, p.mixed ? 1u : 0u};
}

struct DfTrace {
    uint64_t *dev = nullptr;
    size_t words = 0;
    static bool wanted(const std::string &path, long step, long *solves) { return !path.empty() && (*solves)++ == step; }
    int begin(edynhip_ctx *c, size_t n) {
        words = n;
        EH_HIP(c, hipMalloc((void **)&dev, words * 8));
        EH_HIP(c, hipMemsetAsync(dev, 0, words * 8, c->stream));
        return EDYNHIP_OK;
    }
    int end(edynhip_ctx *c, const std::string &path, bool write, uint32_t na, uint32_t stride, uint32_t sweeps, uint32_t per_wave) {
        if (!dev) return EDYNHIP_OK;
        if (write) {
            std::vector<uint64_t> tr(words); std::vector<uint32_t> keys(na);
            EH_HIP(c, hipStreamSynchronize(c->stream));
            EH_HIP(c, hipMemcpy(tr.data(), dev, words * 8, hipMemcpyDeviceToHost));
            EH_HIP(c, hipMemcpy(keys.data(), c->col_keys_sorted, (size_t)na * 4, hipMemcpyDeviceToHost));
            if (FILE *f = fopen(path.c_str(), "wb")) {
                const uint32_t hdr[4] = {na, stride, sweeps, per_wave};
                fwrite(hdr, 4, 4, f); fwrite(keys.data(), 4, na, f); fwrite(tr.data(), 8, words, f); fclose(f);
            }
        }
        (void)hipFree(dev);
        dev = nullptr;
        return EDYNHIP_OK;
    }
};

static void joints_pass(edynhip_ctx *c, bool warm, uint32_t *launches) {
    hipStream_t s = c->stream;
    const Joints &j = c->j;
    for (uint32_t k = 0; k < j.num_colours; ++k) {
        uint32_t a = j.colour_start[k], e = j.colour_start[k + 1];
        if (e <= a) continue;
        if (warm) hipLaunchKernelGGL(k_joint_solve<true>, dim3(blocks(e - a, 128)), dim3(128), 0, s, a, e, j, c->b);
        else hipLaunchKernelGGL(k_joint_solve<false>, dim3(blocks(e - a, 128)), dim3(128), 0, s, a, e, j, c->b);
        ++*launches;
    }
}
static void contacts_pass(edynhip_ctx *c, const SolvePlan &p, bool warm, uint32_t *launches) {
    hipStream_t s = c->stream;
    const Rows &r = c->rows;
    const uint32_t rcap = c->m[c->cur].cap;
    const bool push = p.push, fused_rows = p.fused_rows;
    for (uint32_t k = 0; k < p.first_tail; ++k) {
        uint32_t a = c->colour_start[k], e = c->colour_end[k];
        if (e <= a) continue;
        const Split sp{c->colour_split[k][0], c->colour_split[k][1], c->colour_split[k][2]};
        const dim3 g(blocks(e - a, 64)), bl(64);
        if (push) hipLaunchKernelGGL(contact_solve_fn(warm, true, fused_rows), g, bl, 0, s, a, e, sp, (const uint32_t *)r.next, (const uint32_t *)nullptr, r.rw, rcap, r.dslot, (const float *)r.im, (float4 *)nullptr);
        else hipLaunchKernelGGL(contact_solve_fn(warm, false, fused_rows), g, bl, 0, s, a, e, sp, (const uint32_t *)r.bA, (const uint32_t *)r.bB, r.rw, rcap, c->b.dvw, (const float *)nullptr, c->extras ? r.rwx : (float4 *)nullptr);
        ++*launches;
    }
    if (p.tail.n) {
        const dim3 g(1), bl(kTailThreads);
        if (push) hipLaunchKernelGGL(contact_tail_fn(warm, true, fused_rows), g, bl, 0, s, p.tail, (const uint32_t *)r.next, (const uint32_t *)nullptr, r.rw, rcap, r.dslot, (const float *)r.im, (float4 *)nullptr);
        else hipLaunchKernelGGL(contact_tail_fn(warm, false, fused_rows), g, bl, 0, s, p.tail, (const uint32_t *)r.bA, (const uint32_t *)r.bB, r.rw, rcap, c->b.dvw, (const float *)nullptr, c->extras ? r.rwx : (float4 *)nullptr);
        ++*launches;
    }
    if (p.serial) {
        const uint32_t a = c->colour_start[kSerialColour], e = c->colour_end[kSerialColour];
        const Split sp{c->colour_split[kSerialColour][0], c->colour_split[kSerialColour][1], c->colour_split[kSerialColour][2]};
        hipLaunchKernelGGL(contact_serial_fn(warm, fused_rows), dim3(1), dim3(64), 0, s, a, e, sp, (const uint32_t *)r.bA, (const uint32_t *)r.bB, r.rw, rcap, c->b.dvw, c->extras ? r.rwx : (float4 *)nullptr);
        ++*launches;
    }
}
static int launch_velocity(edynhip_ctx *c, SolvePlan &p, uint32_t *launches) {
    hipStream_t s = c->stream;
    const Knobs &kn = c->knobs;
    if (p.lanes) {
        const Rows &r = c->rows;
        const uint32_t na = p.na, grid = p.vel_grid, per_wave = 64u / p.lanes;
        const uint32_t xcd_lists = (kn.df_xcd && p.lanes == 2u && grid % kXcds == 0 && grid >= 8 * kXcds) ? 1u : 0u;
        DfArgs a{na, grid * per_wave, c->cfg.num_velocity_iterations + 1, c->col_keys_sorted, r.next, r.im, r.rw, c->m[c->cur].cap, r.dslot, c->cnt, nullptr, p.df_skip(c),
                 (uint32_t)kn.df_nap, xcd_lists};
        DfTrace trace;
        if (DfTrace::wanted(kn.df_trace, kn.df_trace_step, &c->df_solves)) {
            a.xcd_lists = 0;
            const uint32_t rounds = (na + a.stride - 1) / a.stride;
            EH_TRY(trace.begin(c, 4 * (size_t)a.sweeps * rounds * (a.stride / per_wave)));
            a.trace = trace.dev;
        }
        void *params[] = {&a};
        if (launch_resident(c, df_velocity_fn(p.lanes, p.fused_rows), grid, 64, params) == hipSuccess) {
            ++*launches;
            c->paths |= (p.lanes == 4u ? EDYNHIP_PATH_VEL_LANES4 : p.lanes == 2u ? EDYNHIP_PATH_VEL_LANES2 : EDYNHIP_PATH_VEL_LANES1) | (a.xcd_lists ? EDYNHIP_PATH_VEL_XCD : 0u) |
                        (na > a.stride ? EDYNHIP_PATH_VEL_MULTI_ROUND : 0u) | (p.lanes == 2u && a.nap != 1u ? EDYNHIP_PATH_VEL_NAP : 0u);
        } else {
            (void)hipGetLastError();
            c->df_mode = 0;
            p.drop_dataflow();
            if (p.mixed) {
                (void)trace.end(c, kn.df_trace, false, na, a.stride, a.sweeps, per_wave);
                return set_error(c, EDYNHIP_ERR_INTERNAL, "solve: the runtime refused the resident launch of the mixed schedule");
            }
        }
        EH_TRY(trace.end(c, kn.df_trace, p.lanes != 0, na, a.stride, a.sweeps, per_wave));
    }
    if ((!p.lanes && p.isl_fused) || (p.lanes && p.mixed)) {
        c->paths |= p.lanes ? EDYNHIP_PATH_MIXED : EDYNHIP_PATH_ISLAND_FUSED;
        const IslSolveArgs isl_args = island_args(c, p, c->cfg.num_velocity_iterations);
        if (p.fused_rows) hipLaunchKernelGGL(k_island_velocity<true>, dim3(kIslGrid), dim3(64), 0, s, isl_args);
        else hipLaunchKernelGGL(k_island_velocity<false>, dim3(kIslGrid), dim3(64), 0, s, isl_args);
        ++*launches;
    } else if (!p.lanes) {
        if (p.na + c->j.n) c->paths |= EDYNHIP_PATH_PER_COLOUR;
        joints_pass(c, true, launches);
        contacts_pass(c, p, true, launches);
        for (uint32_t it = 0; it < c->cfg.num_velocity_iterations; ++it) {
            joints_pass(c, false, launches);
            contacts_pass(c, p, false, launches);
        }
    }
    return EDYNHIP_OK;
}

static void pos_per_colour(edynhip_ctx *c, const SolvePlan &p, uint32_t first_it) {
    hipStream_t s = c->stream;
    const Joints &j = c->j;
    const Manifolds &mf = c->m[c->cur];
    const uint32_t n = c->b.n;
    const bool block_pos = p.block_pos;
    for (uint32_t it = first_it; it < c->cfg.num_position_iterations; ++it) {
        for (uint32_t k = 0; k < j.num_colours; ++k) {
            uint32_t a = j.colour_start[k], e = j.colour_start[k + 1];
            if (e > a) hipLaunchKernelGGL(k_pos_joints, dim3(blocks(e - a, 128)), dim3(128), 0, s, a, e, j, c->b, c->isl_err, c->isl_done);
        }
        for (uint32_t k = 0; k < p.first_tail; ++k) {
            uint32_t a = c->colour_start[k], e = c->colour_end[k];
            if (e > a) hipLaunchKernelGGL(block_pos ? k_pos_contacts<true> : k_pos_contacts<false>, dim3(blocks(2 * (e - a), 128)), dim3(128), 0, s, a, e, c->rows, mf, c->b, c->isl_err, (const uint32_t *)c->isl_done);
        }
        if (p.tail.n) hipLaunchKernelGGL(block_pos ? k_pos_contacts_tail<true> : k_pos_contacts_tail<false>, dim3(1), dim3(256), 0, s, p.tail, c->rows, mf, c->b, c->isl_err, (const uint32_t *)c->isl_done);
        if (p.serial) hipLaunchKernelGGL(block_pos ? k_pos_contacts_serial<true> : k_pos_contacts_serial<false>, dim3(1), dim3(64), 0, s, c->colour_start[kSerialColour], c->colour_end[kSerialColour], c->rows, mf, c->b, c->isl_err, (const uint32_t *)c->isl_done);
        hipLaunchKernelGGL(k_pos_flags, dim3(blocks(n, 256)), dim3(256), 0, s, n, c->isl_err, c->isl_done);
    }
}
static int launch_position(edynhip_ctx *c, const SolvePlan &p, const float4 **final_pslot) {
    hipStream_t s = c->stream;
    const Knobs &kn = c->knobs;
    const Manifolds &mf = c->m[c->cur];
    const uint32_t n = c->b.n, na = p.na, P = c->cfg.num_position_iterations;
    const bool block_pos = p.block_pos;
    if (p.pos_df) {
        const Rows &r = c->rows;
        const uint32_t grid = p.pos_grid;
        hipLaunchKernelGGL(k_pos_seed, dim3(blocks(2 * na, 256)), dim3(256), 0, s, na, r, c->b, r.pslot, mf.cap, mf, p.df_skip(c));
        const uint32_t prounds = blocks(na, grid * 32u);
        const size_t ptrace_words = 4 * (size_t)prounds * grid;
        DfTrace trace;
        if (DfTrace::wanted(kn.dfp_trace, kn.df_trace_step, &c->dfp_solves)) EH_TRY(trace.begin(c, ptrace_words * P));
        uint32_t it = 0;
        for (; it < P; ++it) {
            const uint32_t xcd_lists = (kn.df_xcd && !trace.dev && grid % kXcds == 0 && grid >= 8 * kXcds) ? 1u : 0u;
            DfPosArgs a{na, grid * 32u, it, c->col_keys_sorted, r.next, r.pslot, r, mf, c->b, c->pos_err + (size_t)it * c->b.cap,
                        it ? c->pos_err + (size_t)(it - 1) * c->b.cap : nullptr, c->cnt, p.df_skip(c), trace.dev ? trace.dev + ptrace_words * it : nullptr, xcd_lists};
            void *params[] = {&a};
            if (launch_resident(c, df_position_fn(block_pos), grid, 64, params) != hipSuccess) {
                (void)hipGetLastError();
                c->df_mode = 0;
                break;
            }
            c->paths |= (xcd_lists ? EDYNHIP_PATH_POS_XCD : 0u) | (na > a.stride ? EDYNHIP_PATH_POS_MULTI_ROUND : 0u);
        }
        EH_TRY(trace.end(c, kn.dfp_trace, true, na, grid * 32u, P, 32u));
        if (it == P) {
            *final_pslot = r.pslot;
            if (p.mixed) {
                const IslSolveArgs isl_args = island_args(c, p, P);
                hipLaunchKernelGGL(block_pos ? k_island_position<true> : k_island_position<false>, dim3(kIslGrid), dim3(64), 0, s, isl_args);
            }
        } else if (p.mixed) {
            return set_error(c, EDYNHIP_ERR_INTERNAL, "solve: the runtime refused the resident launch of the mixed schedule (position)");
        } else {
            hipLaunchKernelGGL(k_pos_writeback, dim3(blocks(n, 256)), dim3(256), 0, s, n, c->b, r.pslot, r.first_slot);
            if (it > 0) hipLaunchKernelGGL(k_pos_flags, dim3(blocks(n, 256)), dim3(256), 0, s, n, c->pos_err + (size_t)(it - 1) * c->b.cap, c->isl_done);
            pos_per_colour(c, p, it);
        }
    } else if (P > 0 && (na || c->j.n)) {
        if (p.isl_fused) {
            const IslSolveArgs isl_args = island_args(c, p, P);
            hipLaunchKernelGGL(block_pos ? k_island_position<true> : k_island_position<false>, dim3(kIslGrid), dim3(64), 0, s, isl_args);
        } else {
            if (p.push) c->paths |= EDYNHIP_PATH_POS_COLOUR_PUSH;
            pos_per_colour(c, p, 0);
        }
    }
    return EDYNHIP_OK;
}

int solve(edynhip_ctx *c) {
    hipStream_t s = c->stream;
    const uint32_t n = c->b.n;
    if (n == 0) return EDYNHIP_OK;
    Manifolds &mf = c->m[c->cur];
    const Joints &j = c->j;
    const float dt = c->cfg.fixed_dt;
    const uint32_t rcap = mf.cap;
    rec(c, 3);
    EH_TRY(restitution(c));
    if (!c->solve_begin_done) hipLaunchKernelGGL(k_solve_begin, dim3(blocks(n, 256)), dim3(256), 0, s, n, c->b, dt, c->rows.first_slot);
    c->solve_begin_done = false;
    if (c->df_mode < 0) probe_dataflow(c, (c->cfg.flags & EDYNHIP_FLAG_FUSED_VELOCITY_ROWS) != 0, (c->cfg.flags & EDYNHIP_FLAG_BLOCK_POSITION) != 0);
    bool spec_prep = false;
    auto speculative_prep = [&]() {
        rec(c, 4);
        if (!(c->knobs.speculate && j.n == 0 && !c->extras && c->df_mode == 1 && c->full_step && c->num_manifolds > 0)) return;
        prep_contacts(c, c->num_manifolds, true, true, kPwInPrep);
        spec_prep = true;
    };
    bool first_final = false;
    EH_TRY(colour_contacts(c, speculative_prep, &first_final));
    if (!first_final) spec_prep = false;
    c->all_asleep = c->sleep_active() && c->full_step && c->num_manifolds > 0 && c->cnt_host->num_awake == 0;
    if (c->num_manifolds == 0) rec(c, 4);
    if (j.n) hipLaunchKernelGGL(k_prep_joints, dim3(blocks(j.n, 128)), dim3(128), 0, s, j, c->b, dt, c->isl_joint);
    if (j.n && c->has_generic) hipLaunchKernelGGL(k_prep_generic, dim3(blocks(j.n, 64)), dim3(64), 0, s, j, c->b, dt);

    SolvePlan p = plan_solve(c);
    const uint32_t na = p.na;

    if (na && !spec_prep) prep_contacts(c, na, p.push, false, !c->extras && kPwInPrep);
    if (p.isl_candidate) EH_TRY(bucket_islands(c, p));
    if (p.push) {
        hipLaunchKernelGGL(k_push_links, dim3(blocks(na, 256)), dim3(256), 0, s, na, c->rows, c->col_keys_sorted, c->b, c->used, p.mixed ? c->isl_joint : nullptr);
    }
    rec(c, 5);

    uint32_t launches = 0;
    EH_TRY(launch_velocity(c, p, &launches));
    c->timings.solve_velocity_launches += launches;
    c->stats.solve_schedule = p.schedule(j.n);
    rec(c, 6);

    hipLaunchKernelGGL(k_integrate, dim3(blocks(n, 256)), dim3(256), 0, s, n, c->b, dt, c->isl_err, c->isl_done, p.push ? c->rows.dslot : nullptr, c->rows.first_slot,
                       c->pos_err, p.pos_df ? c->cfg.num_position_iterations : 0u);
    if (na && !p.pos_df) hipLaunchKernelGGL(k_store_impulses, dim3(blocks(na, 256)), dim3(256), 0, s, na, c->rows, rcap, mf);
    rec(c, 7);

    const float4 *final_pslot = nullptr;
    EH_TRY(launch_position(c, p, &final_pslot));
    rec(c, 8);

    hipLaunchKernelGGL(k_finish, dim3(blocks(n, 256)), dim3(256), 0, s, n, c->b, c->used, c->m[c->cur ^ 1].seg_start, c->m[c->cur ^ 1].seg_end, c->cnt,
                       final_pslot, c->rows.first_slot, CandLists{c->bvh.cand_list, c->bvh.cand_count, c->bvh.ref_min, c->bvh.ref_max}, c->isl_joint, c->isl_top, c->meshes);
    rec(c, 9);
    ++c->step_index;
    EH_HIP(c, hipGetLastError());
    return EDYNHIP_OK;
}

}
```

edyn_amd/world.py:

```python
import ctypes as C
import math
from dataclasses import dataclass, field
from typing import Optional, Sequence
import numpy as np
from . import _capi
from ._capi import EdynHipError, MANIFOLD_DTYPE

KIND_DYNAMIC, KIND_KINEMATIC, KIND_STATIC = 0, 1, 2
SHAPE_NONE, SHAPE_BOX, SHAPE_SPHERE, SHAPE_PLANE, SHAPE_CAPSULE, SHAPE_CYLINDER, SHAPE_POLYHEDRON = 0, 1, 2, 3, 4, 5, 6
JOINT_POINT, JOINT_HINGE, JOINT_DISTANCE, JOINT_SOFT_DISTANCE, JOINT_CONE, JOINT_CVJOINT, JOINT_GRAVITY, JOINT_GENERIC = 0, 1, 2, 3, 4, 5, 6, 7
ALL_GROUPS = 2**64 - 1


@dataclass
class init_config:
    fixed_dt: float = 1.0 / 60.0
    num_solver_velocity_iterations: int = 8
    num_solver_position_iterations: int = 3
    max_steps_per_update: int = 10
    gravity: Sequence[float] = (0.0, -9.8, 0.0)
    device: int = 0
    max_bodies: int = 0
    max_manifolds: int = 0
    max_joints: int = 0
    timing: bool = False
    timing_solve: bool = False
    sleeping: bool = False
    contact_events: bool = False
    exclusive_device: bool = False
    fused_velocity_rows: bool = False
    block_position: bool = False


@dataclass
class rigidbody_def:
    kind: int = KIND_DYNAMIC
    position: Sequence[float] = (0.0, 0.0, 0.0)
    orientation: Sequence[float] = (0.0, 0.0, 0.0, 1.0)
    mass: float = 1.0
    inertia: Optional[Sequence[float]] = None
    linvel: Sequence[float] = (0.0, 0.0, 0.0)
    angvel: Sequence[float] = (0.0, 0.0, 0.0)
    gravity: Optional[Sequence[float]] = None
    shape_type: int = SHAPE_NONE
    shape_param: Sequence[float] = (0.0, 0.0, 0.0, 0.0)
    friction: float = 0.5
    restitution: float = 0.0
    collision_group: int = ALL_GROUPS
    collision_mask: int = ALL_GROUPS
    sleeping_disabled: bool = False


def _ptr(a):
    return None if a is None else a.ctypes.data_as(C.c_void_p)


def fixed_step_plan(accumulated, elapsed, fixed_dt, max_steps):
    accumulated += max(elapsed, 0.0)
    num_steps = int(math.floor(accumulated / fixed_dt))
    advance = num_steps * fixed_dt
    accumulated -= advance
    if num_steps > max_steps:
        return max_steps, accumulated, advance / max_steps
    return num_steps, accumulated, fixed_dt


class World:

    def __init__(self, config: Optional[init_config] = None):
        self.cfg = config or init_config()
        self._h = None
        self._defs = []
        self._joints = []
        self._dirty = True
        self._paused = False
        self._accum = 0.0
        self._last_time = 0.0
        self.n = 0
        self.nj = 0
        self.num_meshes = 0
        self._mesh_sig = []
        self._L = _capi.lib()

    def attach(self, max_bodies, max_joints=0):
        self.detach()
        cfg = _capi.Config()
        cfg.device = self.cfg.device
        cfg.max_bodies = max(int(max_bodies), 1)
        cfg.max_manifolds = int(self.cfg.max_manifolds)
        cfg.max_joints = max(int(max_joints), 0)
        cfg.fixed_dt = self.cfg.fixed_dt
        cfg.num_velocity_iterations = self.cfg.num_solver_velocity_iterations
        cfg.num_position_iterations = self.cfg.num_solver_position_iterations
        cfg.gravity = (C.c_float * 3)(*[float(x) for x in self.cfg.gravity])
        cfg.flags = ((_capi.FLAG_TIMING if self.cfg.timing else 0) | (_capi.FLAG_TIMING_SOLVE if self.cfg.timing_solve else 0)
                     | (_capi.FLAG_SLEEPING if self.cfg.sleeping else 0)
                     | (_capi.FLAG_CONTACT_EVENTS if self.cfg.contact_events else 0)
                     | (_capi.FLAG_EXCLUSIVE_DEVICE if self.cfg.exclusive_device else 0)
                     | (_capi.FLAG_FUSED_VELOCITY_ROWS if self.cfg.fused_velocity_rows else 0)
                     | (_capi.FLAG_BLOCK_POSITION if self.cfg.block_position else 0))
        st = C.c_int(0)
        h = self._L.edynhip_create(C.byref(cfg), C.byref(st))
        if not h:
            raise EdynHipError(st.value, self._L.edynhip_last_error(None).decode())
        self._h = C.c_void_p(h)
        self.num_meshes = 0
        self._mesh_sig = []
        if getattr(self, "_filter_cb", None) is not None:
            self._check(self._L.edynhip_set_pair_filter(self._h, C.cast(self._filter_cb, C.c_void_p), None))

    def detach(self):
        if self._h:
            self._L.edynhip_destroy(self._h)
            self._h = None

    def __del__(self):
        try:
            self.detach()
        except Exception:
            pass

    def _check(self, rc):
        if rc != 0:
            raise EdynHipError(rc, self._L.edynhip_last_error(self._h).decode())

    def make_rigidbody(self, d: rigidbody_def) -> int:
        self._defs.append(d)
        self._dirty = True
        return len(self._defs) - 1

    def make_constraint(self, jtype, body0, body1, pivot0, pivot1, axis0=(1, 0, 0), axis1=(1, 0, 0), params=None) -> int:
        j = (jtype, body0, body1, tuple(pivot0), tuple(pivot1), tuple(axis0), tuple(axis1))
        self._joints.append(j + ((tuple(params),) if params is not None else ()))
        self._dirty = True
        return len(self._joints) - 1

    def _body_arrays(self, scene):
        n = len(scene["kind"])
        a = {}
        a["kind"] = np.ascontiguousarray(scene["kind"], np.int32)
        for k, w in (("pos", 3), ("orn", 4), ("linvel", 3), ("angvel", 3), ("shape_param", 4)):
            a[k] = np.ascontiguousarray(scene[k], np.float32).reshape(n, w)
        for k in ("mass", "friction", "restitution"):
            a[k] = np.ascontiguousarray(scene[k], np.float32)
        a["shape_type"] = np.ascontiguousarray(scene["shape_type"], np.int32)
        a["group"] = np.ascontiguousarray(scene["group"], np.uint64)
        a["mask"] = np.ascontiguousarray(scene["mask"], np.uint64)
        inertia = scene.get("inertia")
        has_inertia = scene.get("has_inertia")
        if inertia is not None and has_inertia is not None:
            a["inertia"] = np.ascontiguousarray(inertia, np.float32).reshape(n, 9)
            a["has_inertia"] = np.ascontiguousarray(has_inertia, np.uint8)
        grav = scene.get("gravity")
        if grav is not None:
            a["gravity"] = np.ascontiguousarray(grav, np.float32).reshape(n, 3)
        if scene.get("sleeping_disabled") is not None:
            a["sleeping_disabled"] = np.ascontiguousarray(scene["sleeping_disabled"], np.uint8)
        if scene.get("com") is not None:
            a["center_of_mass"] = np.ascontiguousarray(scene["com"], np.float32).reshape(n, 3)
        b = _capi.Bodies()
        for f, _ in _capi.Bodies._fields_:
            setattr(b, f, _ptr(a.get(f)))
        return n, a, b

    @staticmethod
    def _joint_arrays(joints):
        jt = np.array([j[0] for j in joints], np.int32)
        jb = np.array([[j[1], j[2]] for j in joints], np.uint32)
        jp = np.array([[j[3], j[4]] for j in joints], np.float32).reshape(-1, 6)
        ja = np.array([[j[5], j[6]] for j in joints], np.float32).reshape(-1, 6)
        jq = np.zeros((len(joints), 10), np.float32)
        for i, j in enumerate(joints):
            if len(j) > 7:
                jq[i, :len(j[7])] = j[7]
        keep = (jt, jb, jp, ja, jq)
        return keep, _capi.Joints(_ptr(jt), _ptr(jb), _ptr(jp), _ptr(ja), _ptr(jq))

    def _upload_joints(self, joints):
        self.nj = len(joints)
        if joints:
            keep, js = self._joint_arrays(joints)
            self._check(self._L.edynhip_set_joints(self._h, len(joints), C.byref(js)))
        else:
# ... 450 lines not shown
```

include/edynhip.h:

```cpp
#ifndef EDYNHIP_H
#define EDYNHIP_H

#include <stddef.h>
#include <stdint.h>

#ifdef __cplusplus
extern "C" {
#endif

typedef struct edynhip_ctx edynhip_ctx;

typedef enum {
    EDYNHIP_OK = 0,
    EDYNHIP_ERR_INVALID = -1,
    EDYNHIP_ERR_NO_DEVICE = -2,
    EDYNHIP_ERR_HIP = -3,
    EDYNHIP_ERR_CAPACITY = -4,
    EDYNHIP_ERR_COLOURS = -5,
    EDYNHIP_ERR_UNSUPPORTED = -6,
    EDYNHIP_ERR_INTERNAL = -7
} edynhip_status;

enum { EDYNHIP_KIND_DYNAMIC = 0, EDYNHIP_KIND_KINEMATIC = 1, EDYNHIP_KIND_STATIC = 2 };
enum { EDYNHIP_SHAPE_NONE = 0, EDYNHIP_SHAPE_BOX = 1, EDYNHIP_SHAPE_SPHERE = 2, EDYNHIP_SHAPE_PLANE = 3,
       EDYNHIP_SHAPE_CAPSULE = 4,
       EDYNHIP_SHAPE_CYLINDER = 5,
       EDYNHIP_SHAPE_POLYHEDRON = 6  };
enum { EDYNHIP_JOINT_POINT = 0, EDYNHIP_JOINT_HINGE = 1,
       EDYNHIP_JOINT_DISTANCE = 2,
       EDYNHIP_JOINT_SOFT_DISTANCE = 3,
       EDYNHIP_JOINT_CONE = 4,
       EDYNHIP_JOINT_CVJOINT = 5,
       EDYNHIP_JOINT_GRAVITY = 6,
       EDYNHIP_JOINT_GENERIC = 7,
       EDYNHIP_JOINT_NULL = 8             };
enum { EDYNHIP_ATTACH_NONE = 0, EDYNHIP_ATTACH_ON_A = 1, EDYNHIP_ATTACH_ON_B = 2 };

typedef struct {
    int32_t device;
    uint32_t max_bodies;
    uint32_t max_manifolds;
    uint32_t max_joints;
    float fixed_dt;
    uint32_t num_velocity_iterations;
    uint32_t num_position_iterations;
    float gravity[3];
    uint32_t flags;
} edynhip_config;

enum {
    EDYNHIP_FLAG_TIMING = 1u,
    EDYNHIP_FLAG_TIMING_SOLVE = 16u,
    EDYNHIP_FLAG_SLEEPING = 4u,
    EDYNHIP_FLAG_CONTACT_EVENTS = 32u,
    EDYNHIP_FLAG_FUSED_VELOCITY_ROWS = 64u,
    EDYNHIP_FLAG_BLOCK_POSITION = 128u,
    EDYNHIP_FLAG_EXCLUSIVE_DEVICE = 8u
};

typedef struct {
    const int32_t *kind;
    const float *pos;
    const float *orn;
    const float *linvel;
    const float *angvel;
    const float *mass;
    const float *inertia;
    const uint8_t *has_inertia;
    const int32_t *shape_type;
    const float *shape_param;
    const float *friction;
    const float *restitution;
    const uint64_t *group;
    const uint64_t *mask;
    const float *gravity;
    const uint8_t *sleeping_disabled;
    const float *center_of_mass;
} edynhip_bodies;

typedef struct {
    const int32_t *type;
    const uint32_t *body;
    const float *pivot;
    const float *axis;
    const float *params;
} edynhip_joints;

typedef struct {
    float fixed_dt;
    uint32_t num_velocity_iterations;
    uint32_t num_position_iterations;
    float gravity[3];
    uint32_t num_restitution_iterations;
    uint32_t num_individual_restitution_iterations;
} edynhip_params;

typedef struct {
    float pivotA[3], pivotB[3], normal[3], local_normal[3];
    float distance, friction, restitution;
    int32_t attachment;
    uint32_t lifetime;
    float normal_impulse, friction_impulse[2];
} edynhip_point;

typedef struct {
    uint32_t body[2];
    uint32_t num_points;
    uint32_t colour;
    edynhip_point pt[4];
} edynhip_manifold;

enum {
    EDYNHIP_STAGE_BROADPHASE = 1u,
    EDYNHIP_STAGE_NARROWPHASE = 2u,
    EDYNHIP_STAGE_ISLANDS = 4u,
    EDYNHIP_STAGE_SOLVE = 8u,
    EDYNHIP_STAGE_ALL = 15u
};

typedef struct {
    float broadphase_ms, narrowphase_ms, islands_ms, colouring_ms, prepare_ms, solve_velocity_ms,
          integrate_ms, solve_position_ms, finish_ms, step_ms;
    uint32_t solve_velocity_launches;
    uint32_t steps;
} edynhip_timings;

typedef struct {
    uint32_t num_bodies, num_manifolds, num_points, num_active_manifolds, num_islands, num_colours,
             num_joint_colours, colour_rounds, num_joints, num_joint_rows;
    uint32_t solve_schedule;
    uint32_t colour_size[64];
} edynhip_stats;

enum {
    EDYNHIP_SCHEDULE_NONE = 0,
    EDYNHIP_SCHEDULE_DATAFLOW2 = 1,
    EDYNHIP_SCHEDULE_DATAFLOW1 = 2,
    EDYNHIP_SCHEDULE_ISLAND_FUSED = 3,
    EDYNHIP_SCHEDULE_MIXED = 4,
    EDYNHIP_SCHEDULE_PER_COLOUR = 5,
    EDYNHIP_SCHEDULE_DATAFLOW4 = 6
};

edynhip_ctx *edynhip_create(const edynhip_config *cfg, int *status_out);
void edynhip_destroy(edynhip_ctx *ctx);
const char *edynhip_last_error(const edynhip_ctx *ctx);

int edynhip_set_stream(edynhip_ctx *ctx, void *hip_stream);

int edynhip_set_bodies(edynhip_ctx *ctx, uint32_t n, const edynhip_bodies *bodies);
int edynhip_set_joints(edynhip_ctx *ctx, uint32_t n, const edynhip_joints *joints);
int edynhip_add_bodies(edynhip_ctx *ctx, uint32_t n, const edynhip_bodies *bodies);

int edynhip_add_joints(edynhip_ctx *ctx, uint32_t n, const edynhip_joints *joints, uint32_t *first_index);
int edynhip_remove_joints(edynhip_ctx *ctx, uint32_t n, const uint32_t *joint_indices);
int edynhip_set_joint_params(edynhip_ctx *ctx, uint32_t joint_index, const float *params10);
int edynhip_remove_bodies(edynhip_ctx *ctx, uint32_t n, const uint32_t *body_indices);
int edynhip_get_params(edynhip_ctx *ctx, edynhip_params *out);
int edynhip_set_params(edynhip_ctx *ctx, const edynhip_params *params);

int edynhip_step(edynhip_ctx *ctx, uint32_t nsteps);
int edynhip_step_timed(edynhip_ctx *ctx, uint32_t nsteps, double first_step_time, double step_dt);
int edynhip_run_stages(edynhip_ctx *ctx, uint32_t stage_mask);
int edynhip_synchronize(edynhip_ctx *ctx);

int edynhip_get_state(edynhip_ctx *ctx, float *pos, float *orn, float *linvel, float *angvel);
int edynhip_set_state(edynhip_ctx *ctx, const float *pos, const float *orn, const float *linvel, const float *angvel);
int edynhip_exclude_collision(edynhip_ctx *ctx, uint32_t body_a, uint32_t body_b);
int edynhip_remove_collision_exclusion(edynhip_ctx *ctx, uint32_t body_a, uint32_t body_b);
typedef int (*edynhip_pair_filter)(void *user, uint32_t body, uint32_t other);
int edynhip_set_pair_filter(edynhip_ctx *ctx, edynhip_pair_filter filter, void *user);
int edynhip_default_should_collide(edynhip_ctx *ctx, uint32_t body_a, uint32_t body_b);
int edynhip_refresh_derived(edynhip_ctx *ctx);
int edynhip_pack_state_device(edynhip_ctx *ctx, void *dst_device, uint32_t first_body, uint32_t count);
int edynhip_get_derived(edynhip_ctx *ctx, float *aabb, float *inertia_world_inv, uint32_t *island);

enum { EDYNHIP_RAYCAST_FEATURE_NONE = 0,
       EDYNHIP_RAYCAST_FEATURE_BOX_FACE = 1,
       EDYNHIP_RAYCAST_FEATURE_CYLINDER_FACE = 2,
       EDYNHIP_RAYCAST_FEATURE_CYLINDER_SIDE_EDGE = 3,
       EDYNHIP_RAYCAST_FEATURE_CAPSULE_HEMISPHERE = 4,
       EDYNHIP_RAYCAST_FEATURE_CAPSULE_SIDE = 5,
       EDYNHIP_RAYCAST_FEATURE_POLYHEDRON_FACE = 6 };
enum { EDYNHIP_RAYCAST_BRUTE_FORCE = 1 };
typedef struct {
    uint32_t body;
    float fraction;
    float normal[3];
    int32_t feature;
    uint32_t feature_index;
    uint32_t reserved;
} edynhip_raycast_hit;
int edynhip_raycast(edynhip_ctx *ctx, uint32_t n, const float *p0, const float *p1, uint32_t num_ignore, const uint32_t *ignore,
                    uint32_t flags, edynhip_raycast_hit *out);
int edynhip_raycast_device(edynhip_ctx *ctx, uint32_t n, const void *p0_f4, const void *p1_f4, uint32_t num_ignore, const uint32_t *ignore,
                           uint32_t flags, void *out);

enum { EDYNHIP_QUERY_PROCEDURAL = 0, EDYNHIP_QUERY_NON_PROCEDURAL = 1, EDYNHIP_QUERY_ISLANDS = 2 };
enum { EDYNHIP_QUERY_BRUTE_FORCE = 1 };
int edynhip_query_aabb(edynhip_ctx *ctx, int category, uint32_t n, const float *boxes6, uint32_t flags,
                       uint32_t *offsets, uint32_t *ids, uint32_t capacity, uint32_t *total);
int edynhip_query_aabb_device(edynhip_ctx *ctx, int category, uint32_t n, const void *boxes_f4, uint32_t flags,
                              void *offsets, void *ids, uint32_t capacity, void *total);
int edynhip_query_aabb_stats(edynhip_ctx *ctx, uint64_t *wave_sorted, uint64_t *wave_filled);

int edynhip_num_manifolds(edynhip_ctx *ctx, uint32_t *n);
int edynhip_get_manifolds(edynhip_ctx *ctx, edynhip_manifold *out, uint32_t capacity, uint32_t *n);
int edynhip_set_manifolds(edynhip_ctx *ctx, const edynhip_manifold *in, uint32_t n);
int edynhip_get_pairs(edynhip_ctx *ctx, uint64_t *keys, uint32_t capacity, uint32_t *n);
int edynhip_get_joint_impulses(edynhip_ctx *ctx, float *impulses10);

int edynhip_set_joint_definition(edynhip_ctx *ctx, uint32_t joint, const float *frame_a9, const float *frame_b9, const float *params16);

int edynhip_set_generic_definition(edynhip_ctx *ctx, uint32_t joint, const float *frame_a9, const float *frame_b9, const float *dof60);
// ... 174 lines not shown
```

Before: 803.9.

## Store lean contact rows and recompute inverse-inertia products in dataflow solvers

Adds a lean row layout in which contact prep stores only three float4 per row. Each manifold's two inverse-inertia matrices and friction coefficients go once into a side array. The dataflow velocity solvers (1, 2 and 4 lanes) load these per manifold and recompute invI·J in registers, cutting the row bytes read from HBM on every sweep. In exchange it adds ALU work and register pressure that could lower occupancy, and more kernel template variants. It is on by default for contact-only solves, with a flag to restore full rows.

Measured after the change: 831.5, median of 6. 3.4% higher.

```diff
diff --git a/edyn_amd/_capi.py b/edyn_amd/_capi.py
--- a/edyn_amd/_capi.py
+++ b/edyn_amd/_capi.py
@@ -45,7 +45,7 @@
 class Stats(C.Structure):
     _fields_ = [(n, C.c_uint32) for n in ("num_bodies", "num_manifolds", "num_points", "num_active_manifolds",
                                           "num_islands", "num_colours", "num_joint_colours", "colour_rounds",
-                                          "num_joints", "num_joint_rows", "solve_schedule")] + [("colour_size", C.c_uint32 * 64)]
+                                          "num_joints", "num_joint_rows", "solve_schedule")] + [("colour_size", C.c_uint32 * 64), ("lean_rows", C.c_uint32)]
 
 
 class WorldStats(C.Structure):
@@ -74,6 +74,7 @@
 
 FLAG_TIMING, FLAG_SLEEPING, FLAG_EXCLUSIVE_DEVICE, FLAG_TIMING_SOLVE, FLAG_CONTACT_EVENTS = 1, 4, 8, 16, 32
 FLAG_FUSED_VELOCITY_ROWS, FLAG_BLOCK_POSITION = 64, 128
+FLAG_FULL_CONTACT_ROWS = 256
 PAIR_FILTER = C.CFUNCTYPE(C.c_int, C.c_void_p, C.c_uint32, C.c_uint32)
 EVENT_DTYPE = np.dtype([("type", np.uint32), ("step", np.uint32), ("body", np.uint32, 2), ("point_id", np.uint64)])
 EVENT_MANIFOLD_CREATED, EVENT_MANIFOLD_DESTROYED, EVENT_POINT_CREATED, EVENT_POINT_DESTROYED = 1, 2, 3, 4
diff --git a/edyn_amd/csrc/capi.hip b/edyn_amd/csrc/capi.hip
--- a/edyn_amd/csrc/capi.hip
+++ b/edyn_amd/csrc/capi.hip
@@ -149,6 +149,7 @@
     Rows &r = c->rows;
     EH_TRY(dalloc(c, r.order, M)); EH_TRY(dalloc(c, r.bA, M)); EH_TRY(dalloc(c, r.bB, M)); EH_TRY(dalloc(c, r.np, M)); EH_TRY(dalloc(c, r.label, M));
     EH_TRY(dalloc(c, r.rw, (size_t)M * kMaxPts * kRowsPerPoint * kRowF));
+    EH_TRY(dalloc(c, r.iw, (size_t)M * 6));
     EH_TRY(dalloc(c, r.dslot, ((size_t)M + 64) * 4));
     EH_TRY(dalloc(c, r.pslot, ((size_t)M + 32) * 6));
     EH_TRY(dalloc(c, r.next, (size_t)M * 2)); EH_TRY(dalloc(c, r.im, (size_t)M * 2));
diff --git a/edyn_amd/csrc/ctx.hpp b/edyn_amd/csrc/ctx.hpp
--- a/edyn_amd/csrc/ctx.hpp
+++ b/edyn_amd/csrc/ctx.hpp
@@ -135,6 +135,7 @@
     uint32_t *slot_of = nullptr;
     uint32_t *first_slot = nullptr;
     uint8_t *skip = nullptr;
+    float4 *iw = nullptr;
 };
 constexpr int kRowF = 5, kRowsPerPoint = 3, kPosF = 4;
 constexpr uint32_t kColUncCap = 16384;
diff --git a/edyn_amd/csrc/solver.hip b/edyn_amd/csrc/solver.hip
--- a/edyn_amd/csrc/solver.hip
+++ b/edyn_amd/csrc/solver.hip
@@ -31,15 +31,17 @@
     if (i < n) solve_begin_body(i, b, dt, first_slot);
 }
 
+template <bool LEAN>
 DI void store_row(float4 *rw, size_t base, size_t cap, f3 Jl, f3 JaA, f3 JaB, float eff, float rhs, float imp, float mu,
                   const BRef &A, const BRef &B) {
     rw[base] = to4(Jl, eff);
     rw[base + cap] = to4(JaA, rhs);
     rw[base + 2 * cap] = to4(JaB, imp);
+    if (LEAN) return;
     rw[base + 3 * cap] = to4(mul(A.inv_I, JaA), mu);
     rw[base + 4 * cap] = to4(mul(B.inv_I, JaB), kLarge);
 }
-template <bool EXTRAS>
+template <bool EXTRAS, bool LEAN>
 __global__ void k_prep_contacts(uint32_t n_active, Rows rows, uint32_t rcap, Manifolds mf, Bodies b, float dt,
                                 const uint32_t *__restrict__ keys_sorted, bool push, bool by_key, bool write_pw) {
     uint32_t p = blockIdx.x * blockDim.x + threadIdx.x;
@@ -56,6 +58,14 @@
         if (is_dynamic(b.flags[ib])) rows.slot_of[(size_t)ib * kMaxColours + col] = 2 * p + 1;
     }
     const BRef A = load_bref(b, ia), B = load_bref(b, ib);
+    if (LEAN) {
+        float mus[kMaxPts];
+#pragma unroll
+        for (uint32_t k = 0; k < (uint32_t)kMaxPts; ++k) mus[k] = k < np ? mf.pB[pt_at(mf.cap, k, m)].w : 0.0f;
+        float4 *iw = rows.iw + p;
+        iw[0] = to4(A.inv_I.r0, mus[0]); iw[rcap] = to4(A.inv_I.r1, mus[1]); iw[2 * (size_t)rcap] = to4(A.inv_I.r2, mus[2]);
+        iw[3 * (size_t)rcap] = to4(B.inv_I.r0, mus[3]); iw[4 * (size_t)rcap] = to4(B.inv_I.r1, 0.0f); iw[5 * (size_t)rcap] = to4(B.inv_I.r2, 0.0f);
+    }
     for (uint32_t k = 0; k < np; ++k) {
         const size_t s = slot_at(mf.cap, k, m), t = pt_at(mf.cap, k, m);
         const float4 a4 = mf.pA[t], b4 = mf.pB[t], n4 = mf.nrm[t], im = mf.imp[t];
@@ -88,7 +98,7 @@
         const float rhs0 = -rel_speed(t0, K1, -t0, K3, A.v, A.w, B.v, B.w);
         const float rhs1 = -rel_speed(t1, L1, -t1, L3, A.v, A.w, B.v, B.w);
         const size_t base = (size_t)(k * kRowsPerPoint) * kRowF * rcap + p, rstride = (size_t)kRowF * rcap;
-        store_row(rows.rw, base, rcap, n, J1, J3, effn, rhsn, im.x, mu, A, B);
+        store_row<LEAN>(rows.rw, base, rcap, n, J1, J3, effn, rhsn, im.x, mu, A, B);
         if (!EXTRAS && push && write_pw) {
             const size_t pb = (size_t)(k * kPosF) * rcap + p;
             rows.pw[pb] = a4; rows.pw[pb + rcap] = b4; rows.pw[pb + 2 * (size_t)rcap] = mf.lnrm[t]; rows.pw[pb + 3 * (size_t)rcap] = n4;
@@ -121,8 +131,8 @@
             }
             if (xm.y > 0) axial(2, n, xi.z, false);
         }
-        store_row(rows.rw, base + rstride, rcap, t0, K1, K3, eff0, rhs0, im.y, 0.0f, A, B);
-        store_row(rows.rw, base + 2 * rstride, rcap, t1, L1, L3, eff1, rhs1, im.z, 0.0f, A, B);
+        store_row<LEAN>(rows.rw, base + rstride, rcap, t0, K1, K3, eff0, rhs0, im.y, 0.0f, A, B);
+        store_row<LEAN>(rows.rw, base + 2 * rstride, rcap, t1, L1, L3, eff1, rhs1, im.z, 0.0f, A, B);
     }
 }
 
@@ -415,6 +425,7 @@
     const uint8_t *skip;
     uint32_t nap;
     uint32_t xcd_lists;
+    const float4 *iw;
 };
 constexpr uint32_t kXcds = 8, kCls = 4 * kMaxColours;
 struct XcdLists { uint32_t pre[kCls + 1]; uint32_t first[kCls], lo[kCls], hi[kCls]; };
@@ -467,15 +478,37 @@
                  "global_store_dwordx4 %0, %2, off offset:1024 sc1" : : "v"(slot), "v"(v), "v"(w) : "memory");
 }
 constexpr uint32_t kDfSpinLimit = 1u << 22;
-template <bool WARM, int NP, bool FUSED>
+template <bool LEAN>
+DI void row_load_df(RowReg &r, const float4 *__restrict__ rw, uint32_t rcap, uint32_t p, int k, int row, const m3 &iA, const m3 &iB) {
+    if (!LEAN) { row_load(r, rw, rcap, p, k, row); return; }
+#pragma unroll
+    for (int f = 0; f < 3; ++f) r.f[f] = rw[(size_t)((k * kRowsPerPoint + row) * kRowF + f) * rcap + p];
+    r.f[3] = to4(mul(iA, from4(r.f[1])), 0.0f);
+    r.f[4] = to4(mul(iB, from4(r.f[2])), 0.0f);
+}
+template <bool WARM, int NP, bool FUSED, bool LEAN>
 DI void df_task(const DfArgs &a, uint32_t p, bool valid, uint32_t np, uint32_t col, uint32_t sweep, uint64_t *trace_slot) {
     constexpr int kEarly = NP > 2 ? 2 : NP;
     RowReg Rn[NP], Rf[NP][2];
     const uint64_t w0 = a.trace ? wall_clock64() : 0;
-#pragma unroll
-    for (int k = 0; k < NP; ++k) row_load(Rn[k], a.rw, a.rcap, p, k, 0);
-#pragma unroll
-    for (int k = 0; k < kEarly; ++k) { row_load(Rf[k][0], a.rw, a.rcap, p, k, 1); row_load(Rf[k][1], a.rw, a.rcap, p, k, 2); }
+    m3 iA = m3_zero(), iB = m3_zero();
+    float mu[NP];
+    if (LEAN) {
+        float4 i4[6];
+#pragma unroll
+        for (int f = 0; f < 6; ++f) i4[f] = a.iw[(size_t)f * a.rcap + p];
+        iA = {from4(i4[0]), from4(i4[1]), from4(i4[2])}; iB = {from4(i4[3]), from4(i4[4]), from4(i4[5])};
+#pragma unroll
+        for (int k = 0; k < NP; ++k) mu[k] = i4[k].w;
+    }
+#pragma unroll
+    for (int k = 0; k < NP; ++k) row_load_df<LEAN>(Rn[k], a.rw, a.rcap, p, k, 0, iA, iB);
+#pragma unroll
+    for (int k = 0; k < kEarly; ++k) { row_load_df<LEAN>(Rf[k][0], a.rw, a.rcap, p, k, 1, iA, iB); row_load_df<LEAN>(Rf[k][1], a.rw, a.rcap, p, k, 2, iA, iB); }
+    if (!LEAN) {
+#pragma unroll
+        for (int k = 0; k < NP; ++k) mu[k] = Rn[k].f[3].w;
+    }
     uint64_t w1 = 0, w2 = 0;
     const uint32_t nA = a.next[2 * (size_t)p], nB = a.next[2 * (size_t)p + 1];
     Delta d;
@@ -508,11 +541,11 @@
             if (a.trace && w2 == 0) w2 = wall_clock64();
             if (mine_now) {
 #pragma unroll
-                for (int k = kEarly; k < NP; ++k) { row_load(Rf[k][0], a.rw, a.rcap, p, k, 1); row_load(Rf[k][1], a.rw, a.rcap, p, k, 2); }
+                for (int k = kEarly; k < NP; ++k) { row_load_df<LEAN>(Rf[k][0], a.rw, a.rcap, p, k, 1, iA, iB); row_load_df<LEAN>(Rf[k][1], a.rw, a.rcap, p, k, 2, iA, iB); }
                 rows_solve_normals<WARM, NP, FUSED>(d, Rn, np);
 #pragma unroll
                 for (int k = 0; k < NP; ++k)
-                    if ((uint32_t)k < np) solve_friction_pair<Lanes1, WARM, FUSED>(d, Rf[k][0], Rf[k][1], Rn[k].f[3].w, Rn[k].f[2].w);
+                    if ((uint32_t)k < np) solve_friction_pair<Lanes1, WARM, FUSED>(d, Rf[k][0], Rf[k][1], mu[k], Rn[k].f[2].w);
                 if (d.imA != 0) df_publish(a.dslot + dslot_at(nA & kSlotMask, 0), d.dvA, d.dwA, sweep + 1);
                 if (d.imB != 0) df_publish(a.dslot + dslot_at(nB & kSlotMask, 0), d.dvB, d.dwB, sweep + 1);
                 if (!WARM) {
@@ -536,7 +569,7 @@
     }
 }
 constexpr uint32_t kDfBlock = 64;
-template <bool FUSED>
+template <bool FUSED, bool LEAN>
 __global__ void __launch_bounds__(kDfBlock) k_contact_solve_df(DfArgs a) {
     const uint32_t t = blockIdx.x * 64u + threadIdx.x;
     const uint32_t rounds = (a.na + a.stride - 1) / a.stride, nwaves = a.stride >> 6;
@@ -550,8 +583,8 @@
             const uint32_t np = 4u - (key & 3u), col = key >> 2;
             const bool big = __any(valid && np > 2);
             uint64_t *tr = a.trace ? a.trace + 4 * ((size_t)(sweep * rounds + round) * nwaves + blockIdx.x) : nullptr;
-            if (sweep == 0) { if (big) df_task<true, 4, FUSED>(a, p, valid, np, col, sweep, tr); else df_task<true, 2, FUSED>(a, p, valid, np, col, sweep, tr); }
-            else { if (big) df_task<false, 4, FUSED>(a, p, valid, np, col, sweep, tr); else df_task<false, 2, FUSED>(a, p, valid, np, col, sweep, tr); }
+            if (sweep == 0) { if (big) df_task<true, 4, FUSED, LEAN>(a, p, valid, np, col, sweep, tr); else df_task<true, 2, FUSED, LEAN>(a, p, valid, np, col, sweep, tr); }
+            else { if (big) df_task<false, 4, FUSED, LEAN>(a, p, valid, np, col, sweep, tr); else df_task<false, 2, FUSED, LEAN>(a, p, valid, np, col, sweep, tr); }
         }
 }
 
@@ -1327,7 +1360,7 @@
     template <bool FUSED> static DI float rhs(const Row2 &r) { return r.rhs; }
     static DI float &imp(Row2 &r) { return r.imp; }
 };
-template <bool WARM, int NP, bool EXACT, bool FUSED>
+template <bool WARM, int NP, bool EXACT, bool FUSED, bool LEAN>
 DI void df2_task(const DfArgs &a, uint32_t p, bool valid, bool sideB, uint32_t np, uint32_t col, uint32_t sweep, uint64_t *trace_slot) {
     Row2 R[NP][kRowsPerPoint];
     float mu[NP];
@@ -1335,6 +1368,12 @@
     const uint32_t slot = 2 * p + (sideB ? 1u : 0u);
     const uint32_t nx = a.next[slot];
     const float im = a.im[slot];
+    float4 i4[3] = {make_float4(0, 0, 0, 0), make_float4(0, 0, 0, 0), make_float4(0, 0, 0, 0)};
+    if (LEAN) {
+#pragma unroll
+        for (int f = 0; f < 3; ++f) i4[f] = a.iw[(size_t)((sideB ? 3 : 0) + f) * a.rcap + p];
+    }
+    const m3 iw = {from4(i4[0]), from4(i4[1]), from4(i4[2])};
 #pragma unroll
     for (int k = 0; k < NP; ++k) {
 #pragma unroll
@@ -1342,15 +1381,15 @@
             const size_t base = (size_t)((k * kRowsPerPoint + r) * kRowF) * a.rcap + p;
             const float4 f0 = a.rw[base];
             const float4 fa = a.rw[base + (size_t)(sideB ? 2 : 1) * a.rcap];
-            const float4 fi = a.rw[base + (size_t)(sideB ? 4 : 3) * a.rcap];
+            const float4 fi = LEAN ? f0 : a.rw[base + (size_t)(sideB ? 4 : 3) * a.rcap];
             Row2 &q = R[k][r];
             const f3 Jl = from4(f0);
             q.jl = sideB ? -Jl : Jl;
             q.ijl = im * q.jl;
-            q.ja = from4(fa); q.ija = from4(fi);
+            q.ja = from4(fa); q.ija = LEAN ? mul(iw, q.ja) : from4(fi);
             q.eff = f0.w;
             q.rhs = FUSED ? dppA(fa.w) * f0.w : dppA(fa.w); q.imp = dppB(fa.w);
-            if (r == 0) mu[k] = dppA(fi.w);
+            if (r == 0) mu[k] = !LEAN ? dppA(fi.w) : k < 3 ? dppA(i4[k < 3 ? k : 0].w) : dppB(i4[0].w);
         }
     }
     Side x;
@@ -1406,15 +1445,15 @@
         }
     }
 }
-template <bool WARM, bool FUSED>
+template <bool WARM, bool FUSED, bool LEAN>
 DI void df2_dispatch(const DfArgs &a, uint32_t p, bool valid, bool sideB, uint32_t np, uint32_t col, uint32_t sweep, uint64_t *tr) {
-    if (!WARM && __all(!valid || np == 4u)) df2_task<WARM, 4, true, FUSED>(a, p, valid, sideB, np, col, sweep, tr);
-    else if (!WARM && __all(!valid || np == 2u)) df2_task<WARM, 2, true, FUSED>(a, p, valid, sideB, np, col, sweep, tr);
-    else if (!WARM && __all(!valid || np == 1u)) df2_task<WARM, 1, true, FUSED>(a, p, valid, sideB, np, col, sweep, tr);
-    else if (__any(np > 2u)) df2_task<WARM, 4, false, FUSED>(a, p, valid, sideB, np, col, sweep, tr);
-    else df2_task<WARM, 2, false, FUSED>(a, p, valid, sideB, np, col, sweep, tr);
-}
-template <bool FUSED>
+    if (!WARM && __all(!valid || np == 4u)) df2_task<WARM, 4, true, FUSED, LEAN>(a, p, valid, sideB, np, col, sweep, tr);
+    else if (!WARM && __all(!valid || np == 2u)) df2_task<WARM, 2, true, FUSED, LEAN>(a, p, valid, sideB, np, col, sweep, tr);
+    else if (!WARM && __all(!valid || np == 1u)) df2_task<WARM, 1, true, FUSED, LEAN>(a, p, valid, sideB, np, col, sweep, tr);
+    else if (__any(np > 2u)) df2_task<WARM, 4, false, FUSED, LEAN>(a, p, valid, sideB, np, col, sweep, tr);
+    else df2_task<WARM, 2, false, FUSED, LEAN>(a, p, valid, sideB, np, col, sweep, tr);
+}
+template <bool FUSED, bool LEAN>
 __global__ void __launch_bounds__(64) k_contact_solve_df2(DfArgs a) {
     const uint32_t t = blockIdx.x * 32u + (threadIdx.x >> 1);
     const bool sideB = threadIdx.x & 1u;
@@ -1431,8 +1470,8 @@
                 const uint32_t p = pt < a.na ? pt : a.na - 1;
                 const uint32_t key = a.keys_sorted[p];
                 const uint32_t np = valid ? 4u - (key & 3u) : 0u, col = key >> 2;
-                if (sweep == 0) df2_dispatch<true, FUSED>(a, p, valid, sideB, np, col, sweep, nullptr);
-                else df2_dispatch<false, FUSED>(a, p, valid, sideB, np, col, sweep, nullptr);
+                if (sweep == 0) df2_dispatch<true, FUSED, LEAN>(a, p, valid, sideB, np, col, sweep, nullptr);
+                else df2_dispatch<false, FUSED, LEAN>(a, p, valid, sideB, np, col, sweep, nullptr);
             }
         return;
     }
@@ -1446,8 +1485,8 @@
             const uint32_t key = a.keys_sorted[p];
             const uint32_t np = valid ? 4u - (key & 3u) : 0u, col = key >> 2;
             uint64_t *tr = a.trace ? a.trace + 4 * ((size_t)(sweep * rounds + round) * nwaves + blockIdx.x) : nullptr;
-            if (sweep == 0) df2_dispatch<true, FUSED>(a, p, valid, sideB, np, col, sweep, tr);
-            else df2_dispatch<false, FUSED>(a, p, valid, sideB, np, col, sweep, tr);
+            if (sweep == 0) df2_dispatch<true, FUSED, LEAN>(a, p, valid, sideB, np, col, sweep, tr);
+            else df2_dispatch<false, FUSED, LEAN>(a, p, valid, sideB, np, col, sweep, tr);
         }
 }
 
@@ -1489,7 +1528,7 @@
     template <bool FUSED> static DI float rhs(const Row4 &r) { return r.rhs; }
     static DI float &imp(Row4 &r) { return r.imp; }
 };
-template <bool WARM, int NP, bool EXACT, bool FUSED>
+template <bool WARM, int NP, bool EXACT, bool FUSED, bool LEAN>
 DI void df4_task(const DfArgs &a, uint32_t p, bool valid, uint32_t role, uint32_t np, uint32_t col, uint32_t sweep, uint64_t *trace_slot) {
     Row4 R[NP][kRowsPerPoint];
     float mu[NP];
@@ -1500,6 +1539,12 @@
     const uint32_t nx = a.next[slot];
     const float im = a.im[slot];
     const size_t off_a = (size_t)(ang ? 1u + side : 0u) * a.rcap, off_i = (size_t)(3u + side) * a.rcap;
+    float4 i4[3] = {make_float4(0, 0, 0, 0), make_float4(0, 0, 0, 0), make_float4(0, 0, 0, 0)};
+    if (LEAN && ang) {
+#pragma unroll
+        for (int f = 0; f < 3; ++f) i4[f] = a.iw[(size_t)(3u * side + (uint32_t)f) * a.rcap + p];
+    }
+    const m3 iw = {from4(i4[0]), from4(i4[1]), from4(i4[2])};
 #pragma unroll
     for (int k = 0; k < NP; ++k) {
 #pragma unroll
@@ -1507,14 +1552,14 @@
             const size_t base = (size_t)((k * kRowsPerPoint + r) * kRowF) * a.rcap + p;
             const float4 fa = a.rw[base + off_a];
             float4 fi = fa;
-            if (ang) fi = a.rw[base + off_i];
+            if (!LEAN && ang) fi = a.rw[base + off_i];
             Row4 &q = R[k][r];
             const f3 Ja = from4(fa);
             q.j = role == 2u ? -Ja : Ja;
             const f3 lin = im * q.j;
-            q.ij = ang ? from4(fi) : lin;
+            q.ij = ang ? (LEAN ? mul(iw, Ja) : from4(fi)) : lin;
             q.eff = qb0(fa.w); q.rhs = FUSED ? qb1(fa.w) * q.eff : qb1(fa.w); q.imp = qb3(fa.w);
-            if (r == 0) mu[k] = qb1(fi.w);
+            if (r == 0) mu[k] = !LEAN ? qb1(fi.w) : k < 3 ? qb1(i4[k < 3 ? k : 0].w) : qb3(i4[0].w);
         }
     }
     f3 x = mk3(0, 0, 0);
@@ -1567,14 +1612,14 @@
         }
     }
 }
-template <bool WARM, bool FUSED>
+template <bool WARM, bool FUSED, bool LEAN>
 DI void df4_dispatch(const DfArgs &a, uint32_t p, bool valid, uint32_t role, uint32_t np, uint32_t col, uint32_t sweep, uint64_t *tr) {
-    if (!WARM && __all(!valid || np == 4u)) df4_task<WARM, 4, true, FUSED>(a, p, valid, role, np, col, sweep, tr);
-    else if (!WARM && __all(!valid || np == 2u)) df4_task<WARM, 2, true, FUSED>(a, p, valid, role, np, col, sweep, tr);
-    else if (__any(np > 2u)) df4_task<WARM, 4, false, FUSED>(a, p, valid, role, np, col, sweep, tr);
-    else df4_task<WARM, 2, false, FUSED>(a, p, valid, role, np, col, sweep, tr);
-}
-template <bool FUSED>
+    if (!WARM && __all(!valid || np == 4u)) df4_task<WARM, 4, true, FUSED, LEAN>(a, p, valid, role, np, col, sweep, tr);
+    else if (!WARM && __all(!valid || np == 2u)) df4_task<WARM, 2, true, FUSED, LEAN>(a, p, valid, role, np, col, sweep, tr);
+    else if (__any(np > 2u)) df4_task<WARM, 4, false, FUSED, LEAN>(a, p, valid, role, np, col, sweep, tr);
+    else df4_task<WARM, 2, false, FUSED, LEAN>(a, p, valid, role, np, col, sweep, tr);
+}
+template <bool FUSED, bool LEAN>
 __global__ void __launch_bounds__(64) __attribute__((amdgpu_waves_per_eu(2, 2))) k_contact_solve_df4(DfArgs a) {
     const uint32_t t = blockIdx.x * 16u + (threadIdx.x >> 2);
     const uint32_t role = threadIdx.x & 3u;
@@ -1588,8 +1633,8 @@
             const uint32_t key = a.keys_sorted[p];
             const uint32_t np = valid ? 4u - (key & 3u) : 0u, col = key >> 2;
             uint64_t *tr = a.trace ? a.trace + 4 * ((size_t)(sweep * rounds + round) * nwaves + blockIdx.x) : nullptr;
-            if (sweep == 0) df4_dispatch<true, FUSED>(a, p, valid, role, np, col, sweep, tr);
-            else df4_dispatch<false, FUSED>(a, p, valid, role, np, col, sweep, tr);
+            if (sweep == 0) df4_dispatch<true, FUSED, LEAN>(a, p, valid, role, np, col, sweep, tr);
+            else df4_dispatch<false, FUSED, LEAN>(a, p, valid, role, np, col, sweep, tr);
         }
 }
 template <int NP, bool BLOCK>
@@ -2313,10 +2358,15 @@
     static const ContactSerialFn t[2][2] = {{k_contact_solve_serial<false, false>, k_contact_solve_serial<false, true>}, {k_contact_solve_serial<true, false>, k_contact_solve_serial<true, true>}};
     return t[warm][fused];
 }
-static const void *df_velocity_fn(uint32_t lanes, bool fused) {
-    if (lanes == 4u) return fused ? (const void *)k_contact_solve_df4<true> : (const void *)k_contact_solve_df4<false>;
-    if (lanes == 2u) return fused ? (const void *)k_contact_solve_df2<true> : (const void *)k_contact_solve_df2<false>;
-    return fused ? (const void *)k_contact_solve_df<true> : (const void *)k_contact_solve_df<false>;
+static const void *df_velocity_fn(uint32_t lanes, bool fused, bool lean) {
+    if (!lean) {
+        if (lanes == 4u) return fused ? (const void *)k_contact_solve_df4<true, false> : (const void *)k_contact_solve_df4<false, false>;
+        if (lanes == 2u) return fused ? (const void *)k_contact_solve_df2<true, false> : (const void *)k_contact_solve_df2<false, false>;
+        return fused ? (const void *)k_contact_solve_df<true, false> : (const void *)k_contact_solve_df<false, false>;
+    }
+    if (lanes == 4u) return fused ? (const void *)k_contact_solve_df4<true, true> : (const void *)k_contact_solve_df4<false, true>;
+    if (lanes == 2u) return fused ? (const void *)k_contact_solve_df2<true, true> : (const void *)k_contact_solve_df2<false, true>;
+    return fused ? (const void *)k_contact_solve_df<true, true> : (const void *)k_contact_solve_df<false, true>;
 }
 static const void *df_position_fn(bool block) { return block ? (const void *)k_pos_contacts_df<true> : (const void *)k_pos_contacts_df<false>; }
 
@@ -2330,7 +2380,7 @@
             int per_cu = 0;
             return hipOccupancyMaxActiveBlocksPerMultiprocessor(&per_cu, fn, kDfBlock, 0) == hipSuccess && per_cu > 0 ? (uint32_t)per_cu * (uint32_t)ncu : 0u;
         };
-        for (uint32_t lanes : {1u, 2u, 4u}) c->df_resident[lanes] = resident(df_velocity_fn(lanes, fused_rows));
+        for (uint32_t lanes : {1u, 2u, 4u}) c->df_resident[lanes] = std::min(resident(df_velocity_fn(lanes, fused_rows, false)), resident(df_velocity_fn(lanes, fused_rows, true)));
         c->dfp_waves = resident(df_position_fn(block_pos));
         if (c->df_resident[1] > 0) c->df_mode = 1;
     }
@@ -2349,11 +2399,12 @@
     bool mixed = false;
     bool isl_fused = false;
     bool push = false;
+    bool lean = false;
     uint32_t lanes = 0, vel_grid = 0;
     bool pos_df = false;
     uint32_t pos_grid = 0;
     void set_largest(uint32_t items) { largest = items; isl_fused = isl_candidate && !mixed && largest <= kIslFusedLimit; }
-    void drop_dataflow() { lanes = 0; pos_df = false; }
+    void drop_dataflow() { lanes = 0; pos_df = false; lean = false; }
     const uint8_t *df_skip(const edynhip_ctx *c) const { return mixed ? c->rows.skip : nullptr; }
     uint32_t schedule(uint32_t num_joints) const {
         return (na + num_joints) == 0 ? EDYNHIP_SCHEDULE_NONE
@@ -2365,6 +2416,7 @@
 constexpr uint32_t kMixedMinFree = 1024;
 constexpr uint32_t kIslGrid = 4096;
 
+static bool lean_rows_wanted(const edynhip_ctx *c) { return !(c->cfg.flags & EDYNHIP_FLAG_FULL_CONTACT_ROWS); }
 static SolvePlan plan_solve(const edynhip_ctx *c) {
     const Knobs &kn = c->knobs;
     const Joints &j = c->j;
@@ -2410,6 +2462,7 @@
         const uint32_t want_waves = kn.df_waves ? (uint32_t)kn.df_waves : std::max(lanes == 4u ? 2048u : lanes == 2u ? 1024u : 512u, blocks(na, per_wave * 9));
         p.lanes = lanes;
         p.vel_grid = std::min(blocks(na, per_wave), std::min(resident, want_waves));
+        p.lean = lean_rows_wanted(c) && contacts_only;
     }
     const uint32_t P = c->cfg.num_position_iterations;
     p.pos_df = P > 0 && P <= kMaxDfPosIters && p.push && c->df_mode == 1 && kn.dataflow_pos && !c->b.com;
@@ -2417,10 +2470,11 @@
     return p;
 }
 
-static void prep_contacts(edynhip_ctx *c, uint32_t count, bool push, bool by_key, bool pw) {
+static void prep_contacts(edynhip_ctx *c, uint32_t count, bool push, bool by_key, bool pw, bool lean) {
     const Manifolds &mf = c->m[c->cur];
-    if (!c->extras) hipLaunchKernelGGL(k_prep_contacts<false>, dim3(blocks(count, 128)), dim3(128), 0, c->stream, count, c->rows, mf.cap, mf, c->b, c->cfg.fixed_dt, c->col_keys_sorted, push, by_key, pw);
-    else hipLaunchKernelGGL(k_prep_contacts<true>, dim3(blocks(count, 128)), dim3(128), 0, c->stream, count, c->rows, mf.cap, mf, c->b, c->cfg.fixed_dt, c->col_keys_sorted, push, by_key, pw);
+    if (!c->extras && !lean) hipLaunchKernelGGL((k_prep_contacts<false, false>), dim3(blocks(count, 128)), dim3(128), 0, c->stream, count, c->rows, mf.cap, mf, c->b, c->cfg.fixed_dt, c->col_keys_sorted, push, by_key, pw);
+    else if (c->extras) hipLaunchKernelGGL((k_prep_contacts<true, false>), dim3(blocks(count, 128)), dim3(128), 0, c->stream, count, c->rows, mf.cap, mf, c->b, c->cfg.fixed_dt, c->col_keys_sorted, push, by_key, pw);
+    else hipLaunchKernelGGL((k_prep_contacts<false, true>), dim3(blocks(count, 128)), dim3(128), 0, c->stream, count, c->rows, mf.cap, mf, c->b, c->cfg.fixed_dt, c->col_keys_sorted, push, by_key, pw);
 }
 
 static int bucket_islands(edynhip_ctx *c, SolvePlan &p) {
@@ -2451,7 +2505,7 @@
         if (p.isl_fused && c->cnt_host->isl_max_items > kIslFusedLimit) p.isl_fused = false;
         if (p.mixed && c->cnt_host->isl_max_jitems > kIslFusedLimit) {
             p.mixed = false; p.push = false; p.drop_dataflow();
-            if (na) prep_contacts(c, na, false, false, false);
+            if (na) prep_contacts(c, na, false, false, false, false);
         }
     }
     return EDYNHIP_OK;
@@ -2535,7 +2589,7 @@
         const uint32_t na = p.na, grid = p.vel_grid, per_wave = 64u / p.lanes;
         const uint32_t xcd_lists = (kn.df_xcd && p.lanes == 2u && grid % kXcds == 0 && grid >= 8 * kXcds) ? 1u : 0u;
         DfArgs a{na, grid * per_wave, c->cfg.num_velocity_iterations + 1, c->col_keys_sorted, r.next, r.im, r.rw, c->m[c->cur].cap, r.dslot, c->cnt, nullptr, p.df_skip(c),
-                 (uint32_t)kn.df_nap, xcd_lists};
+                 (uint32_t)kn.df_nap, xcd_lists, r.iw};
         DfTrace trace;
         if (DfTrace::wanted(kn.df_trace, kn.df_trace_step, &c->df_solves)) {
             a.xcd_lists = 0;
@@ -2544,13 +2598,14 @@
             a.trace = trace.dev;
         }
         void *params[] = {&a};
-        if (launch_resident(c, df_velocity_fn(p.lanes, p.fused_rows), grid, 64, params) == hipSuccess) {
+        if (launch_resident(c, df_velocity_fn(p.lanes, p.fused_rows, p.lean), grid, 64, params) == hipSuccess) {
             ++*launches;
             c->paths |= (p.lanes == 4u ? EDYNHIP_PATH_VEL_LANES4 : p.lanes == 2u ? EDYNHIP_PATH_VEL_LANES2 : EDYNHIP_PATH_VEL_LANES1) | (a.xcd_lists ? EDYNHIP_PATH_VEL_XCD : 0u) |
                         (na > a.stride ? EDYNHIP_PATH_VEL_MULTI_ROUND : 0u) | (p.lanes == 2u && a.nap != 1u ? EDYNHIP_PATH_VEL_NAP : 0u);
         } else {
             (void)hipGetLastError();
             c->df_mode = 0;
+            if (p.lean && na) prep_contacts(c, na, p.push, false, false, false);
             p.drop_dataflow();
             if (p.mixed) {
                 (void)trace.end(c, kn.df_trace, false, na, a.stride, a.sweeps, per_wave);
@@ -2663,11 +2718,12 @@
     if (!c->solve_begin_done) hipLaunchKernelGGL(k_solve_begin, dim3(blocks(n, 256)), dim3(256), 0, s, n, c->b, dt, c->rows.first_slot);
     c->solve_begin_done = false;
     if (c->df_mode < 0) probe_dataflow(c, (c->cfg.flags & EDYNHIP_FLAG_FUSED_VELOCITY_ROWS) != 0, (c->cfg.flags & EDYNHIP_FLAG_BLOCK_POSITION) != 0);
-    bool spec_prep = false;
+    bool spec_prep = false, spec_lean = false;
     auto speculative_prep = [&]() {
         rec(c, 4);
         if (!(c->knobs.speculate && j.n == 0 && !c->extras && c->df_mode == 1 && c->full_step && c->num_manifolds > 0)) return;
-        prep_contacts(c, c->num_manifolds, true, true, kPwInPrep);
+        spec_lean = lean_rows_wanted(c);
+        prep_contacts(c, c->num_manifolds, true, true, kPwInPrep, spec_lean);
         spec_prep = true;
     };
     bool first_final = false;
@@ -2681,7 +2737,7 @@
     SolvePlan p = plan_solve(c);
     const uint32_t na = p.na;
 
-    if (na && !spec_prep) prep_contacts(c, na, p.push, false, !c->extras && kPwInPrep);
+    if (na && (!spec_prep || spec_lean != p.lean)) prep_contacts(c, na, p.push, false, !c->extras && kPwInPrep, p.lean);
     if (p.isl_candidate) EH_TRY(bucket_islands(c, p));
     if (p.push) {
         hipLaunchKernelGGL(k_push_links, dim3(blocks(na, 256)), dim3(256), 0, s, na, c->rows, c->col_keys_sorted, c->b, c->used, p.mixed ? c->isl_joint : nullptr);
@@ -2692,6 +2748,7 @@
     EH_TRY(launch_velocity(c, p, &launches));
     c->timings.solve_velocity_launches += launches;
     c->stats.solve_schedule = p.schedule(j.n);
+    c->stats.lean_rows = p.lean ? 1u : 0u;
     rec(c, 6);
 
     hipLaunchKernelGGL(k_integrate, dim3(blocks(n, 256)), dim3(256), 0, s, n, c->b, dt, c->isl_err, c->isl_done, p.push ? c->rows.dslot : nullptr, c->rows.first_slot,
diff --git a/edyn_amd/world.py b/edyn_amd/world.py
--- a/edyn_amd/world.py
+++ b/edyn_amd/world.py
@@ -30,6 +30,7 @@
     exclusive_device: bool = False
     fused_velocity_rows: bool = False
     block_position: bool = False
+    full_contact_rows: bool = False
 
 
 @dataclass
@@ -98,7 +99,8 @@
                      | (_capi.FLAG_CONTACT_EVENTS if self.cfg.contact_events else 0)
                      | (_capi.FLAG_EXCLUSIVE_DEVICE if self.cfg.exclusive_device else 0)
                      | (_capi.FLAG_FUSED_VELOCITY_ROWS if self.cfg.fused_velocity_rows else 0)
-                     | (_capi.FLAG_BLOCK_POSITION if self.cfg.block_position else 0))
+                     | (_capi.FLAG_BLOCK_POSITION if self.cfg.block_position else 0)
+                     | (_capi.FLAG_FULL_CONTACT_ROWS if self.cfg.full_contact_rows else 0))
         st = C.c_int(0)
         h = self._L.edynhip_create(C.byref(cfg), C.byref(st))
         if not h:
diff --git a/include/edynhip.h b/include/edynhip.h
--- a/include/edynhip.h
+++ b/include/edynhip.h
@@ -55,6 +55,7 @@
     EDYNHIP_FLAG_CONTACT_EVENTS = 32u,
     EDYNHIP_FLAG_FUSED_VELOCITY_ROWS = 64u,
     EDYNHIP_FLAG_BLOCK_POSITION = 128u,
+    EDYNHIP_FLAG_FULL_CONTACT_ROWS = 256u,
     EDYNHIP_FLAG_EXCLUSIVE_DEVICE = 8u
 };
 
@@ -130,6 +131,7 @@
              num_joint_colours, colour_rounds, num_joints, num_joint_rows;
     uint32_t solve_schedule;
     uint32_t colour_size[64];
+    uint32_t lean_rows;
 } edynhip_stats;
 
 enum {
```
